# usamec/GAML

Hardware: AMD Instinct MI355X
Metric: reads_per_sec_scored (higher is better)
Workload: dtype f64; 1 GPU; cfg3: 5 Mbp, 50x 2x150 paired, insert 300+-30; 833333 pairs in all, whole true genome as 1-2 walks, 8 rotating path sets, window cache warm; pairs_total=833333, pairs_per_gpu=833333, genome_bp=5000000, parallelism=reads sharded over 1 GPU(s)

## Files before the change

gaml_amd/api.py:

```python
from __future__ import annotations

import ctypes as C
import importlib.util
import os
import sys

import numpy as np

_HERE = os.path.dirname(os.path.abspath(__file__))
FLAVOUR = os.environ.get("GAML_HIP_FLAVOUR", "release")
LIB_PATH = os.environ.get("GAML_HIP_LIB") or os.path.join(_HERE, "libgaml_hip_dev.so" if FLAVOUR == "dev" else "libgaml_hip.so")

OK, EINVAL, ENODEVICE, EHIP, ESTATE = 0, -1, -2, -3, -4

_i32p = np.ctypeslib.ndpointer(np.int32, flags="C_CONTIGUOUS")
_i64p = np.ctypeslib.ndpointer(np.int64, flags="C_CONTIGUOUS")
_f64p = np.ctypeslib.ndpointer(np.float64, flags="C_CONTIGUOUS")
_u8p = np.ctypeslib.ndpointer(np.uint8, flags="C_CONTIGUOUS")

ALIGMENT = np.dtype([("position", np.int32), ("edit_dist", np.int32), ("read_id", np.int32), ("orientation", np.int32)])
PACBIO_ALIGMENT = np.dtype([("position", np.int32), ("position_end", np.int32), ("read_id", np.int32), ("pad_", np.int32),
                            ("logprob", np.float64)])


# ... 88 lines not shown
    L.gaml_hip_add_pacbio_fastq.argtypes = [vp, C.POINTER(SingleCfg), C.c_char_p]
    L.gaml_hip_set_shard.argtypes = [vp, C.c_int32, C.c_int32]
    L.gaml_hip_set_presharded.argtypes = [vp, C.c_int32]
    L.gaml_hip_put_window_records.argtypes = [vp, C.c_int, C.c_int, _i32p, C.c_int32, vp, C.c_int64]
    L.gaml_hip_put_pacbio_records.argtypes = [vp, C.c_int, _i32p, C.c_int32, vp, C.c_int64]
    L.gaml_hip_add_pacbio_reads.argtypes = [vp, C.POINTER(SingleCfg), C.c_int32, _u8p, _i64p, C.c_char_p]
    L.gaml_hip_pacbio_missing.argtypes = [vp, C.c_int, _i32p, C.c_int32, _i32p, C.c_int32]
    L.gaml_hip_pacbio_missing.restype = C.c_int32
    L.gaml_hip_pacbio_ingest_sam.argtypes = [vp, C.c_int, _i32p, C.c_int32, C.c_char_p, C.c_int64, C.POINTER(C.c_int64)]
    L.gaml_hip_pacbio_records.argtypes = [vp, C.c_int, _i32p, C.c_int32, vp, C.c_int64]
    L.gaml_hip_pacbio_records.restype = C.c_int64
    L.gaml_hip_pacbio_dp_stats.argtypes = [vp, C.c_int, _f64p]
    if hasattr(L, "gaml_hip_debug_sam_logprob"):
        L.gaml_hip_debug_sam_logprob.argtypes = [vp, C.c_char_p, C.c_int32, C.c_char_p, C.c_int32, C.c_char_p, C.c_int64, C.c_double, C.POINTER(C.c_double), vp, vp, C.c_int32]
    if hasattr(L, "gaml_hip_debug_sam_shape"):
        L.gaml_hip_debug_sam_shape.argtypes = [C.c_char_p, C.c_int64, C.c_int32, _i32p, C.c_void_p, C.c_int32]
    if hasattr(L, "gaml_hip_debug_sam_band"):
        L.gaml_hip_debug_sam_band.argtypes = [C.c_char_p, C.c_int64, C.c_int32, _i32p, _i32p, _i32p, _i32p, C.c_int32]
        L.gaml_hip_debug_sam_band.restype = C.c_int32
    L.gaml_hip_calc_prob.argtypes = [vp, _i32p, _i64p, C.c_int32, C.POINTER(C.c_double), _i32p, C.POINTER(C.c_int32)]
    L.gaml_hip_calc_prob_batch.argtypes = [vp, C.c_int32, _i32p, _i64p, _i32p, _f64p, vp, vp]
    L.gaml_hip_calc_partials.argtypes = [vp, _i32p, _i64p, C.c_int32, _f64p, C.POINTER(C.c_int32)]
    L.gaml_hip_combine_partials.argtypes = [vp, _f64p, C.c_int32, C.POINTER(C.c_double), _i32p]
    L.gaml_hip_calc_partials_async.argtypes = [vp, _i32p, _i64p, C.c_int32, vp, vp, C.POINTER(C.c_int32)]
    L.gaml_hip_eval_begin.argtypes = [vp, _i32p, _i64p, C.c_int32, C.POINTER(C.c_int64), C.POINTER(C.c_int32)]
    L.gaml_hip_eval_pending_maxpos.argtypes = [vp, vp, C.c_int64]
    L.gaml_hip_eval_pending_maxpos.restype = C.c_int64
    L.gaml_hip_eval_apply_maxpos.argtypes = [vp, _i32p, C.c_int64]
    L.gaml_hip_eval_finish.argtypes = [vp, _f64p]
    L.gaml_hip_eval_finish_async.argtypes = [vp, vp, vp]
    L.gaml_hip_sync.argtypes = [vp]
    L.gaml_hip_compact_tables.argtypes = [vp]
    L.gaml_hip_eval_score_async.argtypes = [vp, vp, vp]
    L.gaml_hip_eval_score_async.restype = C.c_int32
    L.gaml_hip_eval_coverage_export_async.argtypes = [vp, C.c_int32, vp, C.c_int64, C.POINTER(C.c_int64), vp]
    L.gaml_hip_eval_coverage_finish_async.argtypes = [vp, C.c_int32, vp, C.c_int32, C.c_int32, vp]
    L.gaml_hip_eval_pacbio_pending.argtypes = [vp]
    L.gaml_hip_eval_pacbio_pending.restype = C.c_int32
    L.gaml_hip_eval_pacbio_intervals.argtypes = [vp, C.c_int32]
    L.gaml_hip_eval_pacbio_intervals.restype = C.c_int64
    L.gaml_hip_eval_pacbio_export_async.argtypes = [vp, C.c_int32, vp, C.c_int64, vp]
    L.gaml_hip_eval_pacbio_finish_async.argtypes = [vp, C.c_int32, vp, C.c_int64, C.c_int32, vp]
    L.gaml_hip_num_readsets.argtypes = [vp]
    L.gaml_hip_readset_kind.argtypes = [vp, C.c_int]
    L.gaml_hip_readset_reads.argtypes = [vp, C.c_int]
    L.gaml_hip_readset_reads.restype = C.c_int64
    L.gaml_hip_num_nodes.argtypes = [vp]
    L.gaml_hip_node_len.argtypes = [vp, C.c_int32]
    L.gaml_hip_read_probs.argtypes = [vp, C.c_int, _f64p, C.c_int64]
    L.gaml_hip_bad_bases.argtypes = [vp, C.c_int, C.POINTER(C.c_int64)]
    L.gaml_hip_window_count.argtypes = [vp, C.c_int, C.c_int]
    L.gaml_hip_window_count.restype = C.c_int64
    L.gaml_hip_window_records.argtypes = [vp, C.c_int, C.c_int, _i32p, C.c_int32, vp, C.c_int64]
    L.gaml_hip_window_records.restype = C.c_int64
    L.gaml_hip_align_window.argtypes = [vp, C.c_int, C.c_int, _i32p, C.c_int32]
    L.gaml_hip_align_window.restype = C.c_int64
    if hasattr(L, "gaml_hip_debug_prepare"):
        L.gaml_hip_debug_prepare.argtypes = [vp, _i32p, _i64p, C.c_int32]
    if hasattr(L, "gaml_hip_debug_occurrences"):
        L.gaml_hip_debug_occurrences.argtypes = [vp, C.c_int, C.c_int, _i32p, C.c_int64]
    if hasattr(L, "gaml_hip_debug_occurrences"):
        L.gaml_hip_debug_occurrences.restype = C.c_int64
    if hasattr(L, "gaml_hip_debug_table_occurrences"):
        L.gaml_hip_debug_table_occurrences.argtypes = [vp, C.c_int, C.c_int, _i32p, C.c_int64, _i64p]
    if hasattr(L, "gaml_hip_debug_table_occurrences"):
        L.gaml_hip_debug_table_occurrences.restype = C.c_int64
    if hasattr(L, "gaml_hip_debug_window_walk"):
        L.gaml_hip_debug_window_walk.argtypes = [vp, C.c_int, C.c_int, C.c_int32, _i32p, C.c_int32]
    for new, old in (("gaml_hip_pair_classes", "gaml_hip_debug_class_counts"), ("gaml_hip_last_phases", "gaml_hip_debug_profile"),
                     ("gaml_hip_table_stats", "gaml_hip_debug_table_stats")):
        if not hasattr(L, new) and hasattr(L, old):
            setattr(L, new, getattr(L, old))
    L.gaml_hip_pair_classes.argtypes = [vp, C.c_int, _i64p]
    if hasattr(L, "gaml_hip_debug_fold_check"):
        L.gaml_hip_debug_fold_check.argtypes = [vp, C.c_int, _i64p]
    if hasattr(L, "gaml_hip_debug_radix_sort"):
        L.gaml_hip_debug_radix_sort.argtypes = [vp, C.c_void_p, C.c_void_p, C.c_int64, C.c_int, C.c_int, C.c_void_p]
    if hasattr(L, "gaml_hip_debug_tables_check"):
        L.gaml_hip_debug_tables_check.argtypes = [vp, C.c_int, _i64p]
    if hasattr(L, "gaml_hip_debug_static_check"):
        L.gaml_hip_debug_static_check.argtypes = [vp, C.c_int, _i64p]
    if hasattr(L, "gaml_hip_debug_set_knob"):
        L.gaml_hip_debug_set_knob.argtypes = [vp, C.c_int, C.c_int]
    if hasattr(L, "gaml_hip_shm_exchange_open"):
        L.gaml_hip_shm_exchange_open.argtypes = [vp, C.c_char_p, C.c_int32, C.c_int32, C.c_int32]
        L.gaml_hip_shm_allreduce_sum.argtypes = [vp, C.c_void_p, C.c_int32]
        L.gaml_hip_shm_exchange_close.argtypes = [vp, C.c_int32]
    if hasattr(L, "gaml_hip_fetch_async"):
        L.gaml_hip_fetch_async.argtypes = [vp, C.c_void_p, C.c_int32, C.c_void_p]
        L.gaml_hip_fetch_wait.argtypes = [vp, C.c_void_p, C.c_int32]
    if hasattr(L, "gaml_hip_debug_timeline"):
        L.gaml_hip_debug_timeline.argtypes = [vp, C.c_int, C.c_void_p, C.c_int64]
    L.gaml_hip_last_phases.argtypes = [vp, _f64p]
    L.gaml_hip_table_stats.argtypes = [vp, C.c_int, _i64p]
    L.gaml_hip_aligner_stats.argtypes = [vp, C.POINTER(C.c_int64), C.POINTER(C.c_int64), C.POINTER(C.c_double)]
    L.gaml_hip_aligner_stages.argtypes = [vp, _f64p]
    L.gaml_hip_last_timing.argtypes = [vp, _f64p]
    L.gaml_hip_set_event_timing.argtypes = [vp, C.c_int]
    L.gaml_hip_kernel_stats.argtypes = [vp, C.c_int, C.POINTER(C.c_int64), C.POINTER(C.c_double), C.POINTER(C.c_double)]
    return L


_lib = _load()

def lib():
    return _lib


def version() -> str:
    return _lib.gaml_hip_version().decode()


class FlatPaths:

    def __init__(self, paths):
        self.flat, self.offs = _flat(paths)
        self.n = len(paths)
        self.flat_ptr, self.offs_ptr = self.flat.ctypes.data, self.offs.ctypes.data

    def __len__(self):
        return self.n


def _flat(paths):
    if isinstance(paths, FlatPaths):
        return paths.flat, paths.offs
    flat = np.array([x for p in paths for x in p], dtype=np.int32)
    if flat.size == 0:
        flat = np.zeros(1, np.int32)
    offs = np.zeros(len(paths) + 1, dtype=np.int64)
    offs[1:] = np.cumsum([len(p) for p in paths])
    return flat, offs


def comm_unique_id() -> bytes:
    buf = C.create_string_buffer(128)
    rc = _lib.gaml_hip_comm_unique_id(C.cast(buf, C.c_void_p))
    if rc != OK:
        raise GamlHipError(rc, "gaml_hip_comm_unique_id failed (RCCL not loadable?)")
    return buf.raw


class Context:

    def __init__(self, device: int = 0, rank: int = 0, world: int = 1, presharded: int = 1, devices=None):
        self._h = C.c_void_p()
        if devices is not None:
            devs = np.ascontiguousarray(devices, np.int32)
            rc = _lib.gaml_hip_create_multi(C.byref(self._h), devs, len(devs))
            if rc != OK:
                raise GamlHipError(rc, f"gaml_hip_create_multi(devices={list(devs)}) failed")
            device = int(devs[0])
        else:
            rc = _lib.gaml_hip_create(C.byref(self._h), device)
            if rc != OK:
                raise GamlHipError(rc, f"gaml_hip_create(device={device}) failed")
        self.device = device
        if world != 1:
            self._check(_lib.gaml_hip_set_shard(self._h, rank, world))
        elif presharded != 1:
            self._check(_lib.gaml_hip_set_presharded(self._h, presharded))
        self.rank, self.world = rank, world
        self._fast = None
        self._fast_begin = None
        self._fast_combine = None

# ... 326 lines not shown
        _lib.gaml_hip_window_records(self._h, rs, mate, walk, len(walk), out.ctypes.data, n)
        o = out[:n]
        return np.stack([o["position"], o["edit_dist"], o["read_id"], o["orientation"]], axis=1)

    def align_window(self, rs, mate, walk) -> int:
        walk = np.ascontiguousarray(walk, np.int32)
        return _lib.gaml_hip_align_window(self._h, rs, mate, walk, len(walk))

    def debug_prepare(self, paths):
        flat, offs = _flat(paths)
        self._check(_lib.gaml_hip_debug_prepare(self._h, flat, offs, len(paths)))

    def debug_occurrences(self, rs, mate=0) -> np.ndarray:
        n = _lib.gaml_hip_debug_occurrences(self._h, rs, mate, np.zeros(5, np.int32), 0)
        out = np.zeros(5 * max(1, n), np.int32)
        _lib.gaml_hip_debug_occurrences(self._h, rs, mate, out, n)
        return out.reshape(-1, 5)[:n]

    def debug_table_occurrences(self, rs, mate=0):
        info = np.zeros(3, np.int64)
        n = _lib.gaml_hip_debug_table_occurrences(self._h, rs, mate, np.zeros(5, np.int32), 0, info)
        out = np.zeros(5 * max(1, n), np.int32)
        _lib.gaml_hip_debug_table_occurrences(self._h, rs, mate, out, n, info)
        return out.reshape(-1, 5)[:n], {"incremental": bool(info[0]), "incremental_calls": int(info[1]), "full_calls": int(info[2])}

    def debug_window_walk(self, rs, mate, wid) -> list:
        buf = np.zeros(64, np.int32)
        n = _lib.gaml_hip_debug_window_walk(self._h, rs, mate, wid, buf, 64)
        if n > 64:
            buf = np.zeros(n, np.int32)
            _lib.gaml_hip_debug_window_walk(self._h, rs, mate, wid, buf, n)
        return [int(x) for x in buf[:n]]

    def table_stats(self, rs):
        out = np.zeros(10, np.int64)
        self._check(_lib.gaml_hip_table_stats(self._h, rs, out))
        return {"full_rebuilds": int(out[0]), "delta_updates": int(out[1]), "dirty_pairs": int(out[2]), "worker_rebuilds": int(out[3]), "side_stream_rebuilds": int(out[3]),
                "batches_patched": int(out[4]), "batches_full": int(out[5]), "records_left_out": [int(out[6]), int(out[7])], "delta_records_left_out": int(out[8]),
                "static_index_pairs": int(out[9])}

    def aligner_stats(self):
        w, k, us = C.c_int64(), C.c_int64(), C.c_double()
        _lib.gaml_hip_aligner_stats(self._h, C.byref(w), C.byref(k), C.byref(us))
        return {"windows": w.value, "candidates": k.value, "us": us.value}

    def aligner_stages(self):
        out = np.zeros(6, np.float64)
        self._check(_lib.gaml_hip_aligner_stages(self._h, out))
        return {"strings_upload": out[0], "spans_candidates": out[1], "extension": out[2], "hits_d2h": out[3], "sort_file": out[4], "batches": int(out[5])}

    def last_phases(self):
        out = np.zeros(8, np.float64)
        _lib.gaml_hip_last_phases(self._h, out)
        return out

    def debug_timeline(self, rs: int, cap_waves: int = 1 << 16) -> np.ndarray:
        out = np.zeros((cap_waves, 8), np.uint64)
        n = self._check(_lib.gaml_hip_debug_timeline(self._h, rs, out.ctypes.data, cap_waves))
        return out[:n]

    def debug_set_knob(self, knob, value):
        self._check(_lib.gaml_hip_debug_set_knob(self._h, knob, value))

    def debug_fold_check(self, rs):
        out = np.zeros(6, np.int64)
        self._check(_lib.gaml_hip_debug_fold_check(self._h, rs, out))
        return {"records_left_out": [int(out[0]), int(out[1])], "compact_pairs": [int(out[2]), int(out[3])], "records_checked": int(out[4]),
                "violations": int(out[5])}

    def debug_radix_sort(self, keys, vals=None, begin_bit=0, end_bit=64, running_max=False):
        k = np.ascontiguousarray(keys, np.uint64).copy()
        v = None if vals is None else np.ascontiguousarray(vals, np.uint64).copy()
        m = np.zeros(len(k), np.uint64) if running_max else None
        self._check(_lib.gaml_hip_debug_radix_sort(self._h, k.ctypes.data, None if v is None else v.ctypes.data, len(k), begin_bit, end_bit,
                                                   None if m is None else m.ctypes.data))
        return k, v, m

    def debug_static_check(self, rs):
        out = np.zeros(8, np.int64)
        self._check(_lib.gaml_hip_debug_static_check(self._h, rs, out))
        return {"static_pairs": int(out[0]), "other_pairs": int(out[1]), "violations": int(out[2]), "no_record": int(out[3]),
                "different_windows": int(out[4]), "orientation": int(out[5]), "distance": int(out[6]), "edits_or_code": int(out[7])}

    def debug_tables_check(self, rs):
        out = np.zeros(8, np.int64)
        rc = _lib.gaml_hip_debug_tables_check(self._h, rs, out)
        res = {"pairs": int(out[0]), "compact": int(out[1]), "static": int(out[2]), "two": int(out[3]), "four": int(out[4]), "more": int(out[5]),
               "compared": int(out[6]), "mismatches": int(out[7])}
        if rc != 0 and res["compared"] == 0:
            self._check(rc)
        return res

    def debug_block_partials(self, rs, set_index=0):
        sums, zeros, lay = np.zeros(8192, np.float64), np.zeros(8192, np.int32), np.zeros(8, np.int32)
        _lib.gaml_hip_debug_block_partials.argtypes = [C.c_void_p, C.c_int, C.c_int32, _f64p, _i32p, C.c_int32, _i32p]
        n = _lib.gaml_hip_debug_block_partials(self._h, rs, set_index, sums, zeros, 8192, lay)
        return sums[:max(n, 0)].copy(), zeros[:max(n, 0)].copy(), lay.tolist()

    def pair_classes(self, rs):
        out = np.zeros(4, np.int64)
        self._check(_lib.gaml_hip_pair_classes(self._h, rs, out))
        return out

    debug_table_stats, debug_profile, debug_class_counts = table_stats, last_phases, pair_classes

    def last_timing(self):
        out = np.zeros(3, np.float64)
        _lib.gaml_hip_last_timing(self._h, out)
        return {"host_us": out[0], "device_wall_us": out[1], "kernel_us": out[2]}

    def set_event_timing(self, on):
        _lib.gaml_hip_set_event_timing(self._h, int(on))

    def kernel_stats(self, reset=False):
        n, us, b = C.c_int64(), C.c_double(), C.c_double()
        _lib.gaml_hip_kernel_stats(self._h, 1 if reset else 0, C.byref(n), C.byref(us), C.byref(b))
        return {"launches": n.value, "device_us": us.value, "algo_bytes": b.value}


def debug_sam_band(sam_line: str, total_len: int):
    raw = sam_line.encode()
    f = np.zeros(10, np.int32); r0 = np.zeros(1, np.int32)
    n = _lib.gaml_hip_debug_sam_band(raw, len(raw), total_len, f, r0, np.zeros(1, np.int32), np.zeros(1, np.int32), 0)
    if n < 0:
        raise GamlHipError(n, "malformed SAM line")
    lo = np.zeros(n, np.int32); hi = np.zeros(n, np.int32)
    _lib.gaml_hip_debug_sam_band(raw, len(raw), total_len, f, r0, lo, hi, n)
    keys = ["flags", "len", "posstart", "posend", "sstart", "send", "slen", "tstart", "tend", "edit_dist"]
    return dict(zip(keys, (int(x) for x in f))), int(r0[0]), lo, hi


def debug_sam_shape(sam_line: str, total_len: int):
    raw = sam_line.encode()
    f = np.zeros(6, np.int32)
    n = _lib.gaml_hip_debug_sam_shape(raw, len(raw), total_len, f, None, 0)
    if n < 0:
        raise GamlHipError(n, "malformed SAM line")
    ops = np.zeros(max(1, n), np.uint32)
    _lib.gaml_hip_debug_sam_shape(raw, len(raw), total_len, f, ops.ctypes.data, n)
    keys = ["n_ops", "row_f", "col_f", "bl", "el", "max_width"]
    return dict(zip(keys, (int(x) for x in f))), [(int(o) >> 2, "MID"[int(o) & 3]) for o in ops[:n]]
```

gaml_amd/csrc/ctx.hip.h:

```cpp
#pragma once
#include <hip/hip_runtime.h>
#include <hip/hip_ext.h>
#include "radix_sort.hip.h"

#include <algorithm>
#include <atomic>
#include <fcntl.h>
#include <sys/mman.h>
#include <unistd.h>
#include <chrono>
#include <climits>
#include <limits>
#include <cmath>
#include <cstdio>
#include <cstdlib>
#include <cstring>
#include <immintrin.h>
#include <memory>
#include <set>
#include <string>
#include <thread>
#include <vector>

#include "aligner.hip.h"
// ... 162 lines not shown
  DevBuf rec8[2], first[2], extra[2], inl[2], len_code, len12, static_idx, static_val;
  DevBuf slot_of_read, read_of_slot, dirty_of_slot;
  DevBuf cnt;
  bool built = false;
  int64_t class_count[4] = {0, 0, 0, 0}, n0a = 0, extras[2] = {0, 0}, dropped[2] = {0, 0};
  bool keep_dominated = false;
  std::vector<int32_t> read_of_slot_host;
  bool ros_valid = false;
  void release() {
    for (int m = 0; m < 2; m++) { rec8[m].release(); first[m].release(); extra[m].release(); inl[m].release(); }
    len_code.release(); len12.release(); static_idx.release(); static_val.release(); slot_of_read.release(); read_of_slot.release(); dirty_of_slot.release(); cnt.release();
  }
};

struct BuildScratch {
  DevBuf k_in, k_out, k_tmp, v_in, v_tmp, hist, v_sorted[2], rstart[2], rend[2], one[2], cl, sidx, more[2], start[2], tiles, wins[2], peer0;
  PinBuf h_wins[2], h_peer, h_cnt;
  void release() {
    k_in.release(); k_out.release(); k_tmp.release(); v_in.release(); v_tmp.release(); hist.release(); cl.release(); sidx.release(); tiles.release(); peer0.release();
    for (int m = 0; m < 2; m++) { v_sorted[m].release(); rstart[m].release(); rend[m].release(); one[m].release(); more[m].release(); start[m].release(); wins[m].release(); h_wins[m].release(); }
    h_peer.release(); h_cnt.release();
  }
};

struct BuildPlan { int64_t A[2] = {0, 0}; int n_act[2] = {0, 0}; unsigned tiles = 0, none1 = 0, none2 = 0; int ins_n = 0, units = 1; bool empty = true; };

struct TableRebuild {
  bool active = false;
  bool retired = false;
  int next_slice = 0;
  int64_t start_eval = 0;
  TableDev tab;
  hipStream_t stream = nullptr;
  hipEvent_t done = nullptr, mark = nullptr;
  std::vector<std::pair<int32_t, int32_t>> after;
};

struct PairInfo {
  int64_t class_count[4] = {0, 0, 0, 0};
  int64_t n0a = 0;
  std::vector<uint32_t> len_combo;
  int64_t dropped_records[2] = {0, 0};
};

struct PairedSet {
  gaml_paired_cfg cfg;
  ShortMate mate[2];
  PairInfo pt;
  MateDev dev[2];
  TableDev tab;
  TableRebuild rebuild;
  BuildScratch scratch;
  BuildPlan build_plan;
  int64_t async_rebuilds = 0, retired_windows = 0, eval_count = 0;
  DevBuf lcode, len_combo_dev, combo_tabs, memo;
  int memo_codes = 0;
  bool statics_uploaded = false, kernels_warm = false, prereserved = false;
  DevBuf dl_slot, dl_spill, dl_rec[2], sp_rng[2], sp_rec[2], sp_slot, dstate;
  DevBuf dl_bins, dl_bin_count, dl_blk_tot, dl_wlist, dl_stamps;
  PinBuf h_dstate;
  size_t delta_cap = 0, cap_spill = 0, cap_sprec = 0;
  int64_t nd_est = 0, ns_est = 0;
  bool spill_may_grow = false;
  int dl_seq = 0;
  int64_t full_rebuilds = 0, delta_updates = 0;
  int quiet_calls = 0;
  int64_t delta_left_out = 0, delta_left_out_base = 0;
  bool compact_requested = false;
  PinBuf h_timeline; int timeline_waves = 0;
  PinBuf h_part_sum, h_part_zero;
  size_t host_part_stride = 0;
  int last_total_blocks = 0, last_sets = 1;
  int last_blocks[8] = {0, 0, 0, 0, 0, 0, 0, 0};
  bool last_host_partials = false;
  DevBuf probs, tabs, cov_bits, bad;
  Arena arena;
  struct Persist {
    void* dev = nullptr; size_t bytes = 0;
    size_t cap_w[2] = {0, 0}, cap_lo[2] = {0, 0}, cap_m[2] = {0, 0};
    size_t off_tfloor = 0, off_occ[2] = {0, 0}, off_lo[2] = {0, 0}, off_m[2] = {0, 0};
    bool valid = false;
    void release() { if (dev) (void)hipFree(dev); dev = nullptr; bytes = 0; valid = false; }
  } persist;
  int64_t batches_patched = 0, batches_full = 0;
  size_t batch_slack = 0;
  hipEvent_t ev_tables = nullptr, ev_ovf = nullptr;
  PairedPlanner planner;
  OccImage image[2];
  std::vector<Occ> scratch_occ[2];
  Reducer red;
  Staging stage_pool;
  std::vector<double> ins_tab, floor_tab, logfloor_tab, covthr_tab;
  bool floor_positive = true;
  bool tabs_uploaded = false;
  int64_t last_bad_bases = 0;
};

struct SingleSet {
  gaml_single_cfg cfg;
  ShortMate mate;
  ReadMajor rm;
  MateDev dev;
  DevBuf lens, probs, tabs, occ_arena;
  std::vector<Occ> last_occ;
  Reducer red;
  std::vector<double> floor_tab, logfloor_tab;
  bool tabs_uploaded = false;
  Staging stage;
};

struct DpDev {
  DevBuf path, jobs, ops, scratch, out, dbg;
  void release() { path.release(); jobs.release(); ops.release(); scratch.release(); out.release(); dbg.release(); }
};

struct PbSweepDev {
  DevBuf iv_off, iv;
  std::vector<int32_t> iv_off_host;
  uint64_t generation = ~0ull;
  DevBuf in, all;
  DevBuf key_begin, key_end, pos, key_begin_s, key_end_s, pos_s, end_max, tmp, bad;
  Staging stage;
  void release() {
    iv_off.release(); iv.release(); in.release(); all.release(); key_begin.release(); key_end.release(); pos.release();
    key_begin_s.release(); key_end_s.release(); pos_s.release(); end_max.release(); tmp.release(); bad.release();
    for (int k = 0; k < kRing; k++) { stage.host[k].release(); if (stage.done[k]) (void)hipEventDestroy(stage.done[k]); stage.done[k] = nullptr; stage.armed[k] = false; }
  }
};

struct PacbioSet {
  gaml_single_cfg cfg;
  int64_t n_global = 0, lo = 0, hi = 0;
  std::vector<int32_t> lens;
  double log_match = 0, log_mismatch = 0;
  std::unordered_map<Walk, int32_t, WalkHasher> walk_id;
  std::vector<std::vector<gaml_pacbio_aligment>> recs;
  uint64_t generation = 0, uploaded_generation = ~0ull;
  int32_t max_len = 0;
  int64_t misses = 0;
  DevBuf d_lens, rec_off, rec_walk, rec_logp, walk_count, logprobs;
  Reducer red;
  int64_t last_bad_bases = 0;
  Staging stage;
  PbSweepDev sweep;
  bool have_reads = false;
  std::string bases;
  std::vector<int64_t> base_off;
  std::unordered_map<std::string, int32_t> name_id;
  DevBuf d_bases;
  DpDev dp;
  bool bases_uploaded = false;
  double dp_stats[8] = {0, 0, 0, 0, 0, 0, 0, 0};
};

struct PairedPrep {
  int64_t assembled_records = 0;
  std::vector<int32_t> path_base, start_off, starts;
  int32_t total_bits = 0, n_paths = 0;
  bool general = false;
};

struct SetRef { int kind, idx; };

}
}

using namespace gaml;
using namespace gaml::detail;

struct gaml_hip_ctx {
  gaml::MultiState* multi = nullptr;
  gaml::CommState* comm = nullptr;
  int device = -1;
  DevBuf warm_buf; bool general_warm = false;
  AlnJob aln_job[2];
  hipStream_t stream = nullptr;
  hipStream_t aux_stream = nullptr;
  GraphStore g;
  bool have_graph = false;
  std::vector<std::unique_ptr<SingleSet>> singles;
  std::vector<std::unique_ptr<PairedSet>> paireds;
  std::vector<std::unique_ptr<PacbioSet>> pacbios;
  std::vector<SetRef> handles;
  int32_t rank = 0, world = 1;
  AlignScratch aln_scratch;
  AlignSmall aln_small[2];
  int64_t aln_windows = 0, aln_candidates = 0;
  double aln_us = 0;
  double aln_stage_us[5] = {0, 0, 0, 0, 0};
  int64_t aln_batches = 0;
  int knobs[24] = {0};
  bool direct_write = false;
  int32_t peers = 1;
  std::string err;
  bool event_timing = false;
  int event_every = 1;
  int64_t event_tick = 0;
  std::vector<std::pair<hipEvent_t, hipEvent_t>> ev_pool;
  std::vector<uint64_t> ev_call;
  uint64_t eval_serial = 0;
  size_t ev_used = 0;
  double t_host_us = 0, t_dev_wall_us = 0, t_kernel_us = 0;
  int64_t stat_launches = 0;
  double stat_device_us = 0, stat_algo_bytes = 0;
  DevBuf packed;
  PinBuf packed_host;
  char* shm_base = nullptr; size_t shm_bytes = 0; int shm_rank = 0, shm_world = 0, shm_cap = 0; unsigned long long shm_step = 0; std::string shm_name;
  PinBuf fetch_host;
  unsigned long long fetch_seq = 0;
  hipStream_t fetch_stream = nullptr;
  DevBuf batch_dev;
  PinBuf batch_host;
  bool pending_open = false;
  std::vector<Walk> pending_paths;
  bool pending_paths_valid = false;
  int32_t pending_total_len = 0;
  std::vector<std::unique_ptr<PairedPrep>> pending_prep;
  double pending_host_us = 0;
  double prof[8] = {0, 0, 0, 0, 0, 0, 0, 0};
  bool used_default_stream = false;
  double* status_dst = nullptr; double status_a = 0, status_b = 0; bool status_done = false;
  bool host_results = false;
  bool defer_cov = false;
  struct PendingCov { int paired_idx; CovArgs args; double* out4; };
  std::vector<PendingCov> pending_cov;
  struct PendingPacbio {
    int pacbio_idx;
    double* out4;
    int32_t n_paths;
    int64_t n_node, n_own;
  };
  std::vector<PendingPacbio> pending_pb;
};
```

gaml_amd/csrc/debug_api.hip.h:

```cpp
#pragma once

int gaml_hip_debug_prepare(gaml_hip_ctx* c, const int32_t* flat, const int64_t* offs, int32_t n_paths) {
  if (!c || n_paths < 0 || (n_paths > 0 && (!flat || !offs))) return fail(c, GAML_HIP_EINVAL, "bad arguments");
  if (c->multi) {
    for (int k = 0; k < gaml::multi_num_shards(c->multi); k++)
      if (int e = gaml_hip_debug_prepare(gaml::multi_shard(c->multi, k), flat, offs, n_paths)) return fail(c, e, gaml_hip_last_error(gaml::multi_shard(c->multi, k)));
    return GAML_HIP_OK;
  }
  if (!c->have_graph) return fail(c, GAML_HIP_ESTATE, "no graph set");
  std::vector<Walk> paths = unflatten(flat, offs, n_paths);
  for (auto& h : scoring_order(c)) {
    if (h.kind == 0) { std::vector<Occ> occs; prepare_single_host(c, *c->singles[h.idx], paths, occs); }
    else if (h.kind == 1) {
      PairedPrep p;
      PairedSet& ps = *c->paireds[h.idx];
      if (int e = prepare_paired_structure(c, ps, flat, offs, n_paths)) return e;
      if (int e = align_pending_pair(c, ps)) return e;
      prepare_paired_tables_host(c, ps, p);
    }
  }
  if (c->peers == 1) {
    for (ShortMate* m : filter_mates(c)) m->unsynced.clear();
  }
  return GAML_HIP_OK;
}

int64_t gaml_hip_debug_occurrences(gaml_hip_ctx* c, int rs, int mate, int32_t* out5, int64_t cap) {
  MULTI_SHARD0(c);
  if (!c || rs < 0 || rs >= (int)c->handles.size()) return -1;
  SetRef h = c->handles[rs];
  const std::vector<Occ>* v = nullptr;
  if (h.kind == 0) v = &c->singles[h.idx]->last_occ;
  else if (h.kind == 1 && (mate == 0 || mate == 1)) { PairedSet& ps = *c->paireds[h.idx]; ps.planner.flat_occurrences(mate, ps.scratch_occ[mate]); v = &ps.scratch_occ[mate]; }
  if (!v) return -1;
  for (int64_t i = 0; i < (int64_t)v->size() && i < cap; i++) {
    const Occ& o = (*v)[i];
    out5[5 * i] = o.wid; out5[5 * i + 1] = o.shift; out5[5 * i + 2] = o.min_pos; out5[5 * i + 3] = o.path; out5[5 * i + 4] = o.rank;
  }
  return (int64_t)v->size();
}

int64_t gaml_hip_debug_table_occurrences(gaml_hip_ctx* c, int rs, int mate, int32_t* out5, int64_t cap, int64_t* info3) {
  MULTI_SHARD0(c);
  if (!c || rs < 0 || rs >= (int)c->handles.size() || c->handles[rs].kind != 1 || (mate != 0 && mate != 1)) return -1;
  PairedSet& ps = *c->paireds[c->handles[rs].idx];
  if (info3) { info3[0] = ps.planner.last_was_incremental(); info3[1] = (int64_t)ps.planner.incremental_calls; info3[2] = (int64_t)ps.planner.full_calls; }
  std::vector<Occ> v;
  ps.image[mate].dump(v);
  const std::vector<int32_t>& slots = ps.planner.slots();
  std::unordered_map<int32_t, int32_t> pos;
  for (size_t k = 0; k < slots.size(); k++) pos[slots[k]] = (int32_t)k;
  for (Occ& o : v) { auto it = pos.find(o.path); o.path = it == pos.end() ? -1 : it->second; }
  std::sort(v.begin(), v.end(), [](const Occ& a, const Occ& b) { return a.path != b.path ? a.path < b.path : (a.rank != b.rank ? a.rank < b.rank : a.wid < b.wid); });
  for (int64_t i = 0; i < (int64_t)v.size() && i < cap; i++) {
    const Occ& o = v[(size_t)i];
    out5[5 * i] = o.wid; out5[5 * i + 1] = o.shift; out5[5 * i + 2] = o.min_pos; out5[5 * i + 3] = o.path; out5[5 * i + 4] = o.rank;
  }
  return (int64_t)v.size();
}

int32_t gaml_hip_debug_window_walk(gaml_hip_ctx* c, int rs, int mate, int32_t wid, int32_t* out, int32_t cap) {
  MULTI_SHARD0(c);
  ShortMate* m = mate_of(c, rs, mate);
  if (!m || wid < 0 || wid >= (int32_t)m->win_walk.size()) return -1;
  const Walk& w = *m->win_walk[wid];
  for (int32_t i = 0; i < (int32_t)w.size() && i < cap; i++) out[i] = w[i];
  return (int32_t)w.size();
}



int gaml_hip_debug_timeline(gaml_hip_ctx* c, int rs, unsigned long long* out, int64_t cap_waves) {
  MULTI_SHARD0(c);
  if (!c || rs < 0 || rs >= (int)c->handles.size() || c->handles[rs].kind != 1 || !out) return fail(c, GAML_HIP_EINVAL, "bad arguments");
  PairedSet& s = *c->paireds[c->handles[rs].idx];
  if (!s.h_timeline.p) return 0;
  const int64_t n = std::min<int64_t>(cap_waves, s.timeline_waves);
  memcpy(out, s.h_timeline.p, (size_t)n * 8 * sizeof(unsigned long long));
  return (int)n;
}

int gaml_hip_debug_set_knob(gaml_hip_ctx* c, int knob, int value) {
  if (!c || knob < 0 || knob >= 24) return GAML_HIP_EINVAL;
  if (c->multi) { for (int k = 0; k < gaml::multi_num_shards(c->multi); k++) gaml::multi_shard(c->multi, k)->knobs[knob] = value; return GAML_HIP_OK; }
  c->knobs[knob] = value;
  return GAML_HIP_OK;
}


static void paired_base_records(const PairTables& pt, int32_t slot, int mt, std::vector<RecQuad>& out) {
  const int64_t n0s = pt.class_count[0];
  if (slot < n0s) {
    const uint64_t r = pt.rec8[mt][slot];
    if (r != kNoRec8) out.push_back(RecQuad{(int32_t)(r & 0xffffff), (int32_t)((r >> 24) & 0xfffffff), (int32_t)((r >> 52) & 63) | ((int32_t)((r >> 58) & 1) << 8), 0});
  } else {
    const RecQuad& f = pt.rm[mt].first[slot - n0s];
    if (f.wid >= 0) {
      const int cnt1 = 1 + (int)((uint32_t)f.flags >> 9);
      for (int q = 0; q < cnt1; q++) { RecQuad r = q == 0 ? f : pt.rm[mt].extra[f.link + q - 1]; r.flags &= 0x1ff; r.link = 0; out.push_back(r); }
    }
  }
}

int gaml_hip_debug_fold_check(gaml_hip_ctx* c, int rs, int64_t* out6) {
  MULTI_SHARD0(c);
  if (!c || rs < 0 || rs >= (int)c->handles.size() || c->handles[rs].kind != 1 || !out6) return fail(c, GAML_HIP_EINVAL, "bad arguments");
  PairedSet& s = *c->paireds[c->handles[rs].idx];
  for (int mt = 0; mt < 2; mt++) for (const Window& w : s.mate[mt].wins) if (w.first < 0 && w.count > 0) return fail(c, GAML_HIP_ESTATE, "host-only check: some windows' records exist in the device pool only (use gaml_hip_debug_tables_check)");
  PairTables with, without;
  build_pair_tables(s.mate[0], s.mate[1], with, true);
  build_pair_tables(s.mate[0], s.mate[1], without, false);
  int64_t checked = 0, bad = 0;
  const int64_t n = s.mate[0].n_local();
  std::vector<RecQuad> a, b;
  for (int mt = 0; mt < 2; mt++) {
    const ShortMate& m = s.mate[mt];
    for (int64_t read = 0; read < n; read++) {
      a.clear(); b.clear();
      paired_base_records(with, with.slot_of_read[read], mt, a);
      paired_base_records(without, without.slot_of_read[read], mt, b);
      size_t ia = 0;
      for (size_t ib = 0; ib < b.size(); ib++) {
        checked++;
        const RecQuad& r = b[ib];
        if (ia < a.size() && a[ia].wid == r.wid && a[ia].pos == r.pos && a[ia].flags == r.flags) { ia++; continue; }
        const Window& j = m.wins[r.wid];
        bool ok = false;
        if (j.head >= 0) {
          auto it = m.solo_of_node.find(j.head);
          if (it != m.solo_of_node.end() && m.wins[it->second].active)
// ... 88 lines not shown
  if (!s.last_host_partials || set < 0 || set >= kMaxSets) return 0;
  const int n = s.last_blocks[set];
  const double* hs = (const double*)s.h_part_sum.p + (size_t)set * s.host_part_stride;
  const int* hz = (const int*)s.h_part_zero.p + (size_t)set * s.host_part_stride;
  for (int b = 0; b < n && b < cap; b++) { if (sums) sums[b] = hs[b]; if (zeros) zeros[b] = hz[b]; }
  if (layout8) {
    PairedArgs a; GridPlan gp;
    paired_base_args(c, s, a, gp);
    layout8[0] = gp.blocks0a; layout8[1] = gp.blocks0; layout8[2] = a.blocks01; layout8[3] = a.blocks012; layout8[4] = a.main_blocks; layout8[5] = a.total_blocks;
    layout8[6] = 0; layout8[7] = n;
  }
  return n;
}



int gaml_hip_debug_tables_check(gaml_hip_ctx* c, int rs, int64_t* out8) {
  MULTI_SHARD0(c);
  if (!c || rs < 0 || rs >= (int)c->handles.size() || c->handles[rs].kind != 1 || !out8) return fail(c, GAML_HIP_EINVAL, "bad arguments");
  if (c->device < 0) return fail(c, GAML_HIP_ENODEVICE, "host-only context");
  PairedSet& s = *c->paireds[c->handles[rs].idx];
  HIP_TRY(c, hipSetDevice(c->device));
  if (s.rebuild.active) { if (int e = paired_build_continue(c, s, true)) return e; HIP_TRY(c, hipEventSynchronize(s.rebuild.done)); s.rebuild.active = false; s.rebuild.after.clear(); }
  if (int e = prepare_paired_tables(c, s)) return e;
  if (int e = pool_mirror(c, s, c->stream)) return e;
  if (int e = paired_upload_statics(c, s, c->stream)) return e;
  TableDev T;
  if (int e = paired_build_enqueue(c, s, T, c->stream)) return e;
  HIP_TRY(c, hipStreamSynchronize(c->stream));
  if (int e = paired_build_collect(c, s, T)) { T.release(); return e; }
  ShortMate hm[2];
  for (int mt = 0; mt < 2; mt++) {
    const ShortMate& m = s.mate[mt];
    hm[mt].n_global = m.n_global; hm[mt].lo = m.lo; hm[mt].hi = m.hi; hm[mt].lens = m.lens;
    hm[mt].wins = m.wins;
    std::vector<int4> dp((size_t)s.dev[mt].pool_n);
    if (!dp.empty()) HIP_TRY(c, hipMemcpy(dp.data(), s.dev[mt].pool.p, dp.size() * sizeof(int4), hipMemcpyDeviceToHost));
    hm[mt].pool.resize(dp.size());
    for (size_t k = 0; k < dp.size(); k++) hm[mt].pool[k] = gaml_aligment{dp[k].y, dp[k].z & 0xff, dp[k].w, (dp[k].z >> 8) & 1};
    for (Window& w : hm[mt].wins) w.first = w.dfirst < 0 ? 0 : w.dfirst;
    for (Window& w : hm[mt].wins) if (w.dfirst < 0) { w.count = 0; }
  }
  PairTables pt;
  build_pair_tables(hm[0], hm[1], pt, KNOB(c, 16) != 1, paired_static_ins_n(c, s));
  const int64_t n = s.mate[0].n_local();
  int64_t compared = 0, bad = 0;
  auto fetch = [&](const DevBuf& d, size_t bytes, std::vector<char>& out) -> int {
    out.resize(bytes);
    if (bytes) HIP_TRY(c, hipMemcpy(out.data(), d.p, bytes, hipMemcpyDeviceToHost));
    return 0;
  };
  auto cmp = [&](const DevBuf& d, const void* host, size_t bytes, size_t elem, const char* what) -> int {
    std::vector<char> v;
    if (int e = fetch(d, bytes, v)) return e;
    int64_t b0 = bad;
    for (size_t k = 0; k < bytes / elem; k++) { compared++; if (memcmp(v.data() + k * elem, (const char*)host + k * elem, elem) != 0) bad++; }
    if (bad != b0 && getenv("GAML_HIP_TRACE_HOST")) fprintf(stderr, "tables_check: %s differs in %lld of %zu entries\n", what, (long long)(bad - b0), bytes / elem);
    return 0;
  };
  for (int k = 0; k < 4; k++) { compared++; bad += T.class_count[k] != pt.class_count[k]; }
  compared++; bad += T.n0a != pt.n0a;
  if (bad == 0) {
    const int64_t n0 = pt.class_count[0], n16 = n - n0;
    if (int e = cmp(T.slot_of_read, pt.slot_of_read.data(), (size_t)n * 4, 4, "slot_of_read")) return e;
    if (int e = cmp(T.read_of_slot, pt.read_of_slot.data(), (size_t)n * 4, 4, "read_of_slot")) return e;
    for (int mt = 0; mt < 2; mt++) {
      if (int e = cmp(T.rec8[mt], pt.rec8[mt].data(), (size_t)n0 * 8, 8, "rec8")) return e;
      if (int e = cmp(T.first[mt], pt.rm[mt].first.data(), (size_t)n16 * 16, 16, "first")) return e;
      if (int e = cmp(T.extra[mt], pt.rm[mt].extra.data(), pt.rm[mt].extra.size() * 16, 16, "extra")) return e;
      if (int e = cmp(T.inl[mt], pt.inl[mt].data(), pt.inl[mt].size() * 16, 16, "inl")) return e;
      compared++; bad += T.extras[mt] != (int64_t)pt.rm[mt].extra.size();
      compared++; bad += T.dropped[mt] != pt.dropped_records[mt];
    }
    if (int e = cmp(T.len_code, pt.len_code.data(), (size_t)n0, 1, "len_code")) return e;
    if (int e = cmp(T.static_idx, pt.static_idx.data(), (size_t)pt.n0a * 4, 4, "static_idx")) return e;
    if (int e = cmp(T.len12, pt.len12.data(), (size_t)n16 * 4, 4, "len12")) return e;
    compared++; bad += pt.len_combo != s.pt.len_combo;
  }
  out8[0] = n; out8[1] = T.class_count[0]; out8[2] = T.n0a; out8[3] = T.class_count[1]; out8[4] = T.class_count[2]; out8[5] = T.class_count[3];
  out8[6] = compared; out8[7] = bad;
  T.release();
  return bad ? fail(c, GAML_HIP_ESTATE, "record tables: the device build differs from the host restatement") : GAML_HIP_OK;
}
```

gaml_amd/csrc/gaml_hip.hip:

```cpp
#include "ctx.hip.h"

using namespace gaml;
using namespace gaml::detail;

namespace {

namespace {
struct KernargEnv {
  bool was_set;
  KernargEnv() { was_set = getenv("HIP_FORCE_DEV_KERNARG") != nullptr; setenv("HIP_FORCE_DEV_KERNARG", "1", 0); }
} kernarg_env;
}

int fail(gaml_hip_ctx* c, int code, const std::string& msg) {
  if (c) c->err = msg;
  return code;
}
#define HIP_TRY(c, expr)                                                                      \
  do {                                                                                        \
    hipError_t e__ = (expr);                                                                  \
    if (e__ != hipSuccess)                                                                    \
      return fail(c, GAML_HIP_EHIP, std::string(#expr) + ": " + hipGetErrorString(e__));      \
  } while (0)

// ... 98 lines not shown
  if (c->ev_used == c->ev_pool.size() && c->ev_pool.size() >= 2048) { if (int e = collect_events(c)) return e; }
  if (c->ev_used == c->ev_pool.size()) {
    hipEvent_t a, b;
    HIP_TRY(c, hipEventCreate(&a));
    HIP_TRY(c, hipEventCreate(&b));
    c->ev_pool.emplace_back(a, b);
  }
  if (c->ev_call.size() < c->ev_pool.size()) c->ev_call.resize(c->ev_pool.size(), 0);
  c->ev_call[c->ev_used] = c->eval_serial;
  *out = &c->ev_pool[c->ev_used++];
  return 0;
}

struct OccLayout { size_t direct, multi_off, multi, end; };
OccLayout layout_image(const OccImage& t, size_t at, size_t n_entries = 0) {
  OccLayout l;
  l.direct = at;
  l.multi_off = (l.direct + std::max<size_t>(1, std::max(n_entries, t.occ12.size())) * sizeof(Occ12) + 15) & ~(size_t)15;
  l.multi = (l.multi_off + t.multi_off.size() * sizeof(int32_t) + 15) & ~(size_t)15;
  l.end = (l.multi + std::max<size_t>(1, t.multi.size()) * sizeof(OccQuad) + 15) & ~(size_t)15;
  return l;
}
void pack_image(const OccImage& t, const OccLayout& l, char* base) {
  if (!t.occ12.empty()) memcpy(base + l.direct, t.occ12.data(), t.occ12.size() * sizeof(Occ12));
  const size_t used = l.direct + t.occ12.size() * sizeof(Occ12);
  if (l.multi_off > used) memset(base + used, 0xff, l.multi_off - used);
  memcpy(base + l.multi_off, t.multi_off.data(), t.multi_off.size() * sizeof(int32_t));
  if (!t.multi.empty()) memcpy(base + l.multi, t.multi.data(), t.multi.size() * sizeof(OccQuad));
}
OccLayout layout_occ(const OccTable& t, size_t at) {
  OccLayout l;
  l.direct = at;
  l.multi_off = align16(l.direct + std::max<size_t>(1, t.direct.size()) * sizeof(OccQuad));
  l.multi = align16(l.multi_off + t.multi_off.size() * sizeof(int32_t));
  l.end = align16(l.multi + std::max<size_t>(1, t.multi.size()) * sizeof(OccQuad));
  return l;
}
void pack_occ(const OccTable& t, const OccLayout& l, char* base) {
  if (!t.direct.empty()) memcpy(base + l.direct, t.direct.data(), t.direct.size() * sizeof(OccQuad));
  memcpy(base + l.multi_off, t.multi_off.data(), t.multi_off.size() * sizeof(int32_t));
  if (!t.multi.empty()) memcpy(base + l.multi, t.multi.data(), t.multi.size() * sizeof(OccQuad));
}

int upload_mate(gaml_hip_ctx* c, const ShortMate& m, ReadMajor& rm, MateDev& d, hipStream_t st,
                const std::vector<int32_t>* slot_of_read = nullptr, bool force = false) {
  if (d.pow_n == 0) {
    d.pow_n = m.match_pow.size();
    HIP_TRY(c, d.pows.reserve(2 * d.pow_n * sizeof(double)));
    HIP_TRY(c, hipMemcpy(d.pows.p, m.mismatch_pow.data(), d.pow_n * sizeof(double), hipMemcpyHostToDevice));
    HIP_TRY(c, hipMemcpy(d.pows.as<double>() + d.pow_n, m.match_pow.data(), d.pow_n * sizeof(double), hipMemcpyHostToDevice));
  }
  if (d.uploaded_generation == m.active_generation && !force) return 0;
  build_read_major(m, slot_of_read, rm);
  HIP_TRY(c, hipStreamSynchronize(st));
  HIP_TRY(c, d.first.reserve(std::max<size_t>(1, rm.first.size()) * sizeof(RecQuad)));
  HIP_TRY(c, d.extra.reserve(std::max<size_t>(1, rm.extra.size()) * sizeof(RecQuad)));
  if (!rm.first.empty()) HIP_TRY(c, hipMemcpy(d.first.p, rm.first.data(), rm.first.size() * sizeof(RecQuad), hipMemcpyHostToDevice));
  if (!rm.extra.empty()) HIP_TRY(c, hipMemcpy(d.extra.p, rm.extra.data(), rm.extra.size() * sizeof(RecQuad), hipMemcpyHostToDevice));
  d.uploaded_generation = m.active_generation;
  return 0;
}

MateView view_of(const MateDev& d, const char* arena, const OccLayout& l) {
  MateView v;
  v.first = d.first.as<int4>();
  v.extra = d.extra.as<int4>();
  v.occ = (const int4*)(arena + l.direct);
  v.occ12 = nullptr;
  v.multi_off = (const int*)(arena + l.multi_off);
  v.multi = (const int4*)(arena + l.multi);
  v.mism_pow = d.pows.as<double>();
  v.match_pow = d.pows.as<double>() + d.pow_n;
  return v;
}

std::vector<Walk> unflatten(const int32_t* flat, const int64_t* offs, int32_t n) {
  std::vector<Walk> r(n);
  for (int32_t i = 0; i < n; i++) r[i].assign(flat + offs[i], flat + offs[i + 1]);
  return r;
}

}

#include "paired_launch.hip.h"

namespace {

#include "single_launch.hip.h"
#include "pacbio_launch.hip.h"
#include "aligner_launch.hip.h"
std::vector<ShortMate*> filter_mates(gaml_hip_ctx* c) {
  std::vector<ShortMate*> v;
  for (auto& h : c->handles)
    if (h.kind == 1) { v.push_back(&c->paireds[h.idx]->mate[0]); v.push_back(&c->paireds[h.idx]->mate[1]); }
  return v;
}

int eval_begin(gaml_hip_ctx* c, const int32_t* flat, const int64_t* offs, int32_t n_paths, int64_t* pending) {
  if (!c->have_graph) return fail(c, GAML_HIP_ESTATE, "no graph set");
  if (n_paths < 0 || (n_paths > 0 && (!flat || !offs))) return fail(c, GAML_HIP_EINVAL, "bad path arguments");
  const double t0 = now_us();
  c->eval_serial++;
  for (int32_t i = 0; i < n_paths; i++) if (offs[i + 1] < offs[i]) return fail(c, GAML_HIP_EINVAL, "path offsets must not decrease");
  const bool want_vectors = c->paireds.empty() || !c->singles.empty() || !c->pacbios.empty();
  c->pending_paths_valid = want_vectors;
  if (want_vectors) {
    c->pending_paths.resize((size_t)n_paths);
    for (int32_t i = 0; i < n_paths; i++) c->pending_paths[i].assign(flat + offs[i], flat + offs[i + 1]);
    for (auto& p : c->pending_paths)
      for (int32_t x : p)
        if (x >= c->g.n()) return fail(c, GAML_HIP_EINVAL, "path refers to a node outside the graph");
    c->pending_total_len = 0;
    for (auto& p : c->pending_paths) c->pending_total_len += walk_length(c->g, p);
  }
  if (c->pending_prep.size() != c->paireds.size()) { c->pending_prep.clear(); c->pending_prep.resize(c->paireds.size()); }
  for (size_t i = 0; i < c->paireds.size(); i++) {
    if (!c->pending_prep[i]) c->pending_prep[i].reset(new PairedPrep());
    if (int e = prepare_paired_structure(c, *c->paireds[i], flat, offs, n_paths)) return e;
    if (!want_vectors) c->pending_total_len = c->paireds[i]->planner.total_len();
    const double ta = now_us();
    gpu_probe(c->stream, c->warm_buf.p, "before alignment");
    if (int e = align_pending_pair(c, *c->paireds[i])) return e;
    gpu_probe(c->stream, c->warm_buf.p, "after alignment");
    c->prof[2] = (i ? c->prof[2] : 0.0) + now_us() - ta;
  }
  int64_t n = 0;
  for (ShortMate* m : filter_mates(c)) {
    if (c->peers == 1) m->unsynced.clear();
    n += (int64_t)m->unsynced.size();
  }
  for (auto& s : c->singles) s->mate.unsynced.clear();
  if (pending) *pending = n;
  gpu_probe(c->stream, c->warm_buf.p, "end of eval_begin");
  c->pending_open = true;
  c->pending_host_us = now_us() - t0;
  c->prof[0] = c->pending_host_us;
  return 0;
}

int eval_finish(gaml_hip_ctx* c, void* d_partials, hipStream_t st) {
  if (c->device < 0) return fail(c, GAML_HIP_ENODEVICE, "scoring needs a HIP device: this context is host-only");
  if (!c->pending_open) return fail(c, GAML_HIP_ESTATE, "no evaluation in progress");
  for (ShortMate* m : filter_mates(c))
    if (!m->unsynced.empty())
      return fail(c, GAML_HIP_ESTATE, "sharded context: new windows were aligned; exchange their largest positions "
                                      "(gaml_hip_eval_pending_maxpos -> all-reduce(max) -> gaml_hip_eval_apply_maxpos) before finishing");
  if (c->peers > 1) {
    for (auto& ps : c->paireds)
      if (ps->cfg.penalty_constant > 0 && !c->defer_cov)
        return fail(c, GAML_HIP_ESTATE, "penalty_constant > 0 on a sharded context: the coverage maps of all ranks must be merged "
                                        "(gaml_hip_eval_score_async -> gaml_hip_eval_coverage_export_async -> all-gather -> "
                                        "gaml_hip_eval_coverage_finish_async)");
    for (auto& ps : c->pacbios)
      if (ps->cfg.penalty_constant > 0 && !c->defer_cov)
        return fail(c, GAML_HIP_ESTATE, "penalty_constant > 0 on a sharded PacBio set: the alignment intervals of all ranks must be merged "
                                        "(gaml_hip_eval_score_async -> gaml_hip_eval_pacbio_export_async -> all-gather -> gaml_hip_eval_pacbio_finish_async)");
  }
  const std::vector<Walk>& paths = c->pending_paths;
  const int32_t total_len = c->pending_total_len;
  auto order = scoring_order(c);
  const double t0 = now_us();
  c->t_host_us = 0;
  int k = 0;
  for (auto& h : order) {
    const double tk = now_us();
    double* out4 = (double*)d_partials + 4 * k;
// ... 95 lines not shown
void ctx_eval_abandon(gaml_hip_ctx* c) { if (c) { c->pending_open = false; c->pending_cov.clear(); c->pending_pb.clear(); } }
bool ctx_has_penalty(const gaml_hip_ctx* c) {
  for (auto& ps : c->paireds) if (ps->cfg.penalty_constant > 0) return true;
  for (auto& ps : c->pacbios) if (ps->cfg.penalty_constant > 0) return true;
  return false;
}
}

#define MULTI_FWD(c, call) do { if ((c) && (c)->multi) return gaml::call; } while (0)
#define MULTI_SHARD0(c) do { if ((c) && (c)->multi) (c) = gaml::multi_shard((c)->multi, 0); } while (0)
#define MULTI_REFUSE(c, what) do { if ((c) && (c)->multi) return fail(c, GAML_HIP_ESTATE, "multi-device context: " what); } while (0)

extern "C" {


int gaml_hip_create(gaml_hip_ctx** out, int device) {
  if (!out) return GAML_HIP_EINVAL;
  *out = nullptr;
  std::unique_ptr<gaml_hip_ctx> c(new gaml_hip_ctx());
  c->device = device;
  if (device >= 0) {
    int count = 0;
    hipError_t e = hipGetDeviceCount(&count);
    if (e != hipSuccess || device >= count) {
      fprintf(stderr, "gaml_hip_create: HIP device %d not available (%s)\n", device, e == hipSuccess ? "ordinal out of range" : hipGetErrorString(e));
      return GAML_HIP_ENODEVICE;
    }
    if (hipSetDevice(device) != hipSuccess) return GAML_HIP_EHIP;
    {
      const char* ka = getenv("HIP_FORCE_DEV_KERNARG");
      static bool warned = false;
      if ((!ka || strcmp(ka, "1") != 0) && !warned) {
        warned = true;
        c->err = "HIP_FORCE_DEV_KERNARG is not 1: kernel arguments live in host memory, every scoring launch pays ~4 us for it";
        fprintf(stderr, "libgaml_hip: warning: %s\n", c->err.c_str());
      }
    }
    {
      int lo = 0, hi = 0;
      if (hipDeviceGetStreamPriorityRange(&lo, &hi) != hipSuccess || hipStreamCreateWithPriority(&c->stream, hipStreamNonBlocking, hi) != hipSuccess) return GAML_HIP_EHIP;
    }
    if (hipStreamCreateWithFlags(&c->aux_stream, hipStreamNonBlocking) != hipSuccess) return GAML_HIP_EHIP;
    int large_bar = 0;
    if (hipDeviceGetAttribute(&large_bar, hipDeviceAttributeIsLargeBar, device) != hipSuccess) large_bar = 0;
    const char* dw = getenv("GAML_HIP_DIRECT_WRITE");
    c->direct_write = large_bar != 0 && !(dw && dw[0] == '0');
  }
  *out = c.release();
  return GAML_HIP_OK;
}

void gaml_hip_destroy(gaml_hip_ctx* c) {
#ifdef GAML_GEN_STAMPS
  if (c && c->device >= 0) {
    unsigned long long z[32];
    if (hipMemcpyFromSymbol(z, HIP_SYMBOL(gaml::g_gen_stamp), sizeof(z)) == hipSuccess && z[15]) {
      fprintf(stderr, "general_pair_staged: longest stage us: entries %.1f, bounds %.1f, lists %.1f, liveness %.1f, terms %.1f; waves above 10 us in a stage: %llu %llu %llu %llu %llu\n",
              z[16] * 0.01, z[17] * 0.01, z[18] * 0.01, z[19] * 0.01, z[20] * 0.01, z[24], z[25], z[26], z[27], z[28]);
    }
    if (z[6]) fprintf(stderr, "general_pair_call as the caller sees it: %llu calls, mean %.2f us; from the class body's entry to the call %.2f us\n", z[6], z[5] * 0.01 / z[6], z[21] * 0.01 / z[6]);
    if (z[15])
      fprintf(stderr, "general_pair_staged: %llu waves; mean us per wave: entries %.2f, bounds %.2f, lists %.2f, liveness %.2f, terms %.2f; candidates per lane-0 pair %.1f / %.1f, live %.1f, lanes %.1f; pairs that did not fit %llu; longest %.2f us, most candidates %llu / %llu, most live %llu / %llu\n",
              z[15], z[0] * 0.01 / z[15], z[1] * 0.01 / z[15], z[2] * 0.01 / z[15], z[3] * 0.01 / z[15], z[4] * 0.01 / z[15], (double)z[8] / z[15], (double)z[9] / z[15], (double)z[10] / z[15], (double)z[11] / z[15], z[12], z[13] * 0.01, z[14] / 1000, z[14] % 1000, z[7] / 1000, z[7] % 1000);
  }
#endif
  if (c && c->shm_base) { munmap(c->shm_base, c->shm_bytes); c->shm_base = nullptr; }
  if (!c) return;
  if (c->multi) { gaml::multi_destroy(c->multi); c->multi = nullptr; }
  if (c->device >= 0) {
    (void)hipSetDevice(c->device);
    (void)hipDeviceSynchronize();
    if (c->comm) { gaml::comm_destroy(c->comm); c->comm = nullptr; }
    auto drop_stage = [](Staging& s) { for (int k = 0; k < kRing; k++) { s.host[k].release(); if (s.done[k]) (void)hipEventDestroy(s.done[k]); } };
    for (auto& s : c->singles) { s->dev.first.release(); s->dev.extra.release(); s->dev.pows.release(); s->lens.release(); s->probs.release(); s->tabs.release(); s->occ_arena.release(); s->red.release(); drop_stage(s->stage); }
    for (auto& s : c->paireds) {
      if (s->rebuild.stream) (void)hipStreamDestroy(s->rebuild.stream);
      if (s->rebuild.done) (void)hipEventDestroy(s->rebuild.done);
      if (s->rebuild.mark) (void)hipEventDestroy(s->rebuild.mark);
      s->tab.release(); s->rebuild.tab.release(); s->scratch.release();
      for (int m = 0; m < 2; m++) { s->dev[m].first.release(); s->dev[m].extra.release(); s->dev[m].pows.release(); s->dev[m].aln.release(); s->dev[m].pool.release(); s->dev[m].lens.release();
                                    s->dl_rec[m].release(); s->sp_rng[m].release(); s->sp_rec[m].release(); }
      s->dl_slot.release(); s->dl_spill.release(); s->sp_slot.release(); s->dstate.release(); s->dl_bins.release(); s->dl_bin_count.release(); s->dl_blk_tot.release(); s->dl_wlist.release(); s->h_dstate.release(); s->lcode.release(); s->len_combo_dev.release(); s->combo_tabs.release(); s->memo.release();
      drop_stage(s->stage_pool); s->h_part_sum.release(); s->h_part_zero.release(); s->h_timeline.release();
      s->probs.release(); s->tabs.release(); s->arena.release(); s->persist.release(); s->cov_bits.release(); s->bad.release(); if (s->ev_tables) (void)hipEventDestroy(s->ev_tables); if (s->ev_ovf) (void)hipEventDestroy(s->ev_ovf);
      s->red.release();
    }
    for (auto& s : c->pacbios) { s->d_lens.release(); s->rec_off.release(); s->rec_walk.release(); s->rec_logp.release(); s->walk_count.release(); s->logprobs.release(); s->red.release(); drop_stage(s->stage);
      s->d_bases.release(); s->dp.release(); s->sweep.release(); }
    c->packed.release(); c->packed_host.release(); c->batch_dev.release(); c->batch_host.release(); c->aln_scratch.release();
    c->aln_small[0].release(); c->aln_small[1].release(); c->fetch_host.release(); c->warm_buf.release();
    for (auto& e : c->ev_pool) { (void)hipEventDestroy(e.first); (void)hipEventDestroy(e.second); }
    if (c->stream) (void)hipStreamDestroy(c->stream);
    if (c->aux_stream) (void)hipStreamDestroy(c->aux_stream);
  }
  delete c;
}

const char* gaml_hip_last_error(const gaml_hip_ctx* c) {
  if (!c) return "null context";
  if (c->multi && c->err.empty()) return gaml::multi_last_error(c->multi);
  return c->err.c_str();
}

int gaml_hip_set_graph(gaml_hip_ctx* c, int32_t n_nodes, const char* bases, const int64_t* offs) {
  if (!c || n_nodes < 0 || !offs || (n_nodes > 0 && !bases)) return fail(c, GAML_HIP_EINVAL, "bad graph arguments");
  if (n_nodes & 1) return fail(c, GAML_HIP_EINVAL, "node count must be even (twin of i is i^1)");
  MULTI_FWD(c, multi_set_graph(c->multi, n_nodes, bases, offs));
  c->g.bases.assign(bases + offs[0], bases + offs[n_nodes]);
  c->g.off.resize(n_nodes + 1);
  for (int32_t i = 0; i <= n_nodes; i++) c->g.off[i] = offs[i] - offs[0];
  c->g.finish();
  c->have_graph = true;
  return GAML_HIP_OK;
}

int gaml_hip_load_graph(gaml_hip_ctx* c, const char* file) {
  if (!c || !file) return fail(c, GAML_HIP_EINVAL, "bad arguments");
  MULTI_FWD(c, multi_load_graph(c->multi, file));
  std::string err;
  if (!c->g.load_lastgraph(file, &err)) return fail(c, GAML_HIP_EINVAL, err);
  c->have_graph = true;
  return GAML_HIP_OK;
}

int gaml_hip_set_shard(gaml_hip_ctx* c, int32_t rank, int32_t world) {
  if (!c || world < 1 || rank < 0 || rank >= world) return fail(c, GAML_HIP_EINVAL, "bad shard");
  MULTI_REFUSE(c, "its shards are the devices given to gaml_hip_create_multi");
  if (!c->handles.empty()) return fail(c, GAML_HIP_ESTATE, "set the shard before adding read sets");
  c->rank = rank; c->world = world; c->peers = world;
  return GAML_HIP_OK;
}

int gaml_hip_set_presharded(gaml_hip_ctx* c, int32_t world) {
  if (!c || world < 1) return fail(c, GAML_HIP_EINVAL, "bad arguments");
  MULTI_REFUSE(c, "its shards are the devices given to gaml_hip_create_multi");
  if (c->world != 1) return fail(c, GAML_HIP_ESTATE, "gaml_hip_set_shard already partitions this context's reads");
  c->peers = world;
  return GAML_HIP_OK;
}

static void init_mate(gaml_hip_ctx* c, ShortMate& m, double mismatch, int64_t n, const char* b, const int64_t* offs) {
  m.mismatch = mismatch;
  m.match = 1.0 - 4 * mismatch;
  int64_t lo, hi;
  shard_range(c, n, &lo, &hi);
  m.set_reads(n, lo, hi, b, offs);
}

int gaml_hip_add_single(gaml_hip_ctx* c, const gaml_single_cfg* cfg, int32_t n, const char* bases, const int64_t* offs) {
  if (!c || !cfg || n < 0 || !offs) return fail(c, GAML_HIP_EINVAL, "bad arguments");
  MULTI_FWD(c, multi_add_single(c->multi, cfg, n, bases, offs));
  std::unique_ptr<SingleSet> s(new SingleSet());
  s->cfg = *cfg;
  init_mate(c, s->mate, cfg->mismatch_prob, n, bases, offs);
  c->singles.push_back(std::move(s));
  c->handles.push_back(SetRef{0, (int)c->singles.size() - 1});
  return (int)c->handles.size() - 1;
}

static int warm_general_kernels(gaml_hip_ctx* c) {
  if (c->general_warm || c->device < 0) return 0;
  HIP_TRY(c, hipSetDevice(c->device));
  HIP_TRY(c, c->warm_buf.reserve(256));
  HIP_TRY(c, hipMemsetAsync(c->warm_buf.p, 0, 256, c->stream));
  PairedArgs a;
  memset((void*)&a, 0, sizeof(a));
  a.total_blocks = 1;
// ... 370 lines not shown
  MULTI_REFUSE(c, "no single device to fetch from");
  if (c->device < 0) return fail(c, GAML_HIP_ENODEVICE, "no device");
  HIP_TRY(c, hipSetDevice(c->device));
  const size_t bytes = 512 + (size_t)n_doubles * sizeof(double);
  if (bytes > c->fetch_host.cap) {
    HIP_TRY(c, c->fetch_host.reserve(bytes));
    memset(c->fetch_host.p, 0, c->fetch_host.cap);
  }
  c->fetch_stream = caller_stream(c, stream);
  c->fetch_seq++;
  char* dev = (char*)c->fetch_host.dev;
  hipLaunchKernelGGL(fetch_kernel, dim3(1), dim3(64), 0, c->fetch_stream, (const double*)d_src, (int)n_doubles, (double*)(dev + 512),
                     (unsigned long long*)dev, c->fetch_seq);
  HIP_TRY(c, hipGetLastError());
  return GAML_HIP_OK;
}

int gaml_hip_fetch_wait(gaml_hip_ctx* c, double* out, int32_t n_doubles) {
  if (!c || !out || n_doubles <= 0 || !c->fetch_host.p) return fail(c, GAML_HIP_EINVAL, "bad arguments / no fetch in flight");
  volatile unsigned long long* word = (volatile unsigned long long*)c->fetch_host.p;
  const double t0 = now_us();
  bool seen = false;
  while (now_us() - t0 < 2000.0) {
    for (int k = 0; k < 64 && !seen; k++) seen = *word == c->fetch_seq;
    if (seen) break;
  }
  if (!seen) {
    HIP_TRY(c, hipSetDevice(c->device));
    HIP_TRY(c, hipStreamSynchronize(c->fetch_stream));
    if (*word != c->fetch_seq) return fail(c, GAML_HIP_ESTATE, "fetch kernel finished without publishing its sequence word");
  }
  std::atomic_thread_fence(std::memory_order_acquire);
  memcpy(out, (const char*)c->fetch_host.p + 512, (size_t)n_doubles * sizeof(double));
  return GAML_HIP_OK;
}

int gaml_hip_sync(gaml_hip_ctx* c) {
  MULTI_FWD(c, multi_sync(c->multi));
  if (!c || c->device < 0) return fail(c, GAML_HIP_ENODEVICE, "no device");
  HIP_TRY(c, hipSetDevice(c->device));
  HIP_TRY(c, hipStreamSynchronize(c->stream));
  if (c->used_default_stream) { HIP_TRY(c, hipStreamSynchronize(nullptr)); c->used_default_stream = false; }
  for (auto& ps : c->paireds) paired_refresh_counts(*ps);
  return GAML_HIP_OK;
}

static int fetch_partials(gaml_hip_ctx* c, double* partials_out);

int gaml_hip_eval_finish(gaml_hip_ctx* c, double* partials_out) {
  if (!c || !partials_out) return fail(c, GAML_HIP_EINVAL, "bad arguments");
  MULTI_REFUSE(c, "the gaml_hip_eval_* protocol is for one shard per process");
  if (c->device < 0) return fail(c, GAML_HIP_ENODEVICE, "scoring needs a HIP device: this context is host-only");
  HIP_TRY(c, hipSetDevice(c->device));
  const size_t bytes = std::max<size_t>(1, c->handles.size()) * 4 * sizeof(double);
  HIP_TRY(c, c->packed_host.reserve(bytes));
  void* dres = nullptr;
  HIP_TRY(c, hipHostGetDevicePointer(&dres, c->packed_host.p, 0));
  c->host_results = true;
  int e = eval_finish(c, dres, c->stream);
  c->host_results = false;
  if (e) return e;
  return fetch_partials(c, partials_out);
}

int gaml_hip_calc_partials_async(gaml_hip_ctx* c, const int32_t* paths, const int64_t* offs, int32_t n_paths,
                                 void* d_partials, void* stream, int32_t* total_len_out) {
  if (!c || !d_partials) return fail(c, GAML_HIP_EINVAL, "bad arguments");
  MULTI_REFUSE(c, "partials of several devices have no single device address; use gaml_hip_calc_partials");
  if (c->device >= 0) HIP_TRY(c, hipSetDevice(c->device));
  return evaluate(c, paths, offs, n_paths, d_partials, caller_stream(c, stream), total_len_out);
}

int gaml_hip_calc_partials(gaml_hip_ctx* c, const int32_t* paths, const int64_t* offs, int32_t n_paths,
                           double* partials_out, int32_t* total_len_out) {
  if (!c || !partials_out) return fail(c, GAML_HIP_EINVAL, "bad arguments");
  MULTI_FWD(c, multi_calc_partials(c->multi, paths, offs, n_paths, partials_out, total_len_out));
  if (c->device < 0) return fail(c, GAML_HIP_ENODEVICE, "scoring needs a HIP device: this context is host-only");
  HIP_TRY(c, hipSetDevice(c->device));
  const size_t bytes = std::max<size_t>(1, c->handles.size()) * 4 * sizeof(double);
  HIP_TRY(c, c->packed_host.reserve(bytes));
  void* dres = nullptr;
  HIP_TRY(c, hipHostGetDevicePointer(&dres, c->packed_host.p, 0));
  c->host_results = true;
  int e = evaluate(c, paths, offs, n_paths, dres, c->stream, total_len_out);
  c->host_results = false;
  if (e) return e;
  return fetch_partials(c, partials_out);
}

static void finisher_order_sum(const double* ps, const int* pz, int n, double* sum_out, double* zeros_out) {
  double v[kBlock];
  long long z = 0;
  for (int t = 0; t < kBlock; t++) { double a = 0; for (int b = t; b < n; b += kBlock) a += ps[b]; v[t] = a; }
  for (int b = 0; b < n; b++) z += pz[b];
  double total = 0;
  for (int w = 0; w < kBlock / 64; w++) {
    double* l = v + 64 * w;
    for (int off = 32; off > 0; off >>= 1) for (int i = 0; i < off; i++) l[i] += l[i + off];
    total += l[0];
  }
  *sum_out = total;
  *zeros_out = (double)z;
}

static int wait_host_partials(gaml_hip_ctx* c, bool* spun) {
  const double t0 = now_us();
  bool spin = KNOB(c, 7) == 0 && !c->handles.empty();
  for (auto& h : c->handles) if (h.kind != 1) spin = false;
  for (auto& ps : c->paireds) if (ps->cfg.penalty_constant > 0 || !ps->last_host_partials || ps->last_total_blocks == 0) spin = false;
  if (spin) {
    const double deadline = t0 + 2e6;
    for (auto& ps : c->paireds) {
      for (int k = 0; k < ps->last_sets && spin; k++) {
        const volatile double* hs = (const volatile double*)ps->h_part_sum.p + (size_t)k * ps->host_part_stride;
        const volatile int* hz = (const volatile int*)ps->h_part_zero.p + (size_t)k * ps->host_part_stride;
        int done = 0;
        while (done < ps->last_blocks[k]) {
          if (hs[done] == hs[done] && hz[done] != INT_MIN) { done++; continue; }
          __builtin_ia32_pause();
          if ((done & 63) == 0 && now_us() > deadline) { spin = false; break; }
        }
      }
      if (!spin) break;
    }
    std::atomic_thread_fence(std::memory_order_acquire);
  }
  if (!spin) HIP_TRY(c, hipStreamSynchronize(c->stream));
  c->t_dev_wall_us += now_us() - t0;
  c->prof[7] = now_us() - t0;
  *spun = spin;
  return 0;
}

static int fetch_partials(gaml_hip_ctx* c, double* partials_out) {
  bool spun = false;
  if (int e = wait_host_partials(c, &spun)) return e;
  {
    double* res = (double*)c->packed_host.p;
    auto ord = scoring_order(c);
    for (size_t k = 0; k < ord.size(); k++) {
      if (ord[k].kind != 1) continue;
      PairedSet& s = *c->paireds[ord[k].idx];
      if (!s.last_host_partials) continue;
      if (s.last_blocks[0] > 0)
        finisher_order_sum((const double*)s.h_part_sum.p, (const int*)s.h_part_zero.p, s.last_blocks[0], &res[4 * k], &res[4 * k + 1]);
      else res[4 * k] = res[4 * k + 1] = 0;
      if (!(s.cfg.penalty_constant > 0) || s.last_total_blocks == 0) res[4 * k + 2] = 0;
      res[4 * k + 3] = (double)s.mate[0].n_local();
    }
  }
  memcpy(partials_out, c->packed_host.p, c->handles.size() * 4 * sizeof(double));
  for (auto& ps : c->paireds) {
    paired_refresh_counts(*ps);
    if (paired_delta_overflowed(*ps)) return fail(c, GAML_HIP_ESTATE, "delta store overflow (spill area); call gaml_hip_compact_tables and evaluate again");
  }
  c->t_kernel_us = 0;
  if (!spun) { if (int e2 = collect_events(c)) return e2; }
  auto order = scoring_order(c);
  for (size_t k = 0; k < order.size(); k++) {
    if (order[k].kind == 1) c->paireds[order[k].idx]->last_bad_bases = (int64_t)partials_out[4 * k + 2];
    else if (order[k].kind == 2) c->pacbios[order[k].idx]->last_bad_bases = (int64_t)partials_out[4 * k + 2];
  }
  return GAML_HIP_OK;
}

#include "paired_batch.hip.h"
int gaml_hip_combine_partials(gaml_hip_ctx* c, const double* partials, int32_t total_len, double* prob_out, int32_t* zeros_out) {
  if (!c || !partials || !prob_out) return fail(c, GAML_HIP_EINVAL, "bad arguments");
  MULTI_FWD(c, multi_combine(c->multi, partials, total_len, prob_out, zeros_out));
  return combine(c, partials, prob_out, zeros_out, total_len);
}

int gaml_hip_calc_prob(gaml_hip_ctx* c, const int32_t* paths, const int64_t* offs, int32_t n_paths,
                       double* prob_out, int32_t* zeros_out, int32_t* total_len_out) {
  if (!c || !prob_out) return fail(c, GAML_HIP_EINVAL, "bad arguments");
  const size_t ns = c->multi ? (size_t)gaml::multi_num_readsets(c->multi) : c->handles.size();
  std::vector<double> partials(std::max<size_t>(1, ns) * 4);
  int32_t tl = 0;
  int e;
  if (!c->multi && c->comm) {
    e = gaml::comm_eval_reduced(c, paths, offs, n_paths, partials.data(), &tl);
  } else {
    if (c->peers != 1)
      return fail(c, GAML_HIP_ESTATE, "sharded context without a communicator: gaml_hip_comm_init_rank first, or use gaml_hip_calc_partials + "
                                      "your own all-reduce + gaml_hip_combine_partials");
    e = gaml_hip_calc_partials(c, paths, offs, n_paths, partials.data(), &tl);
  }
  if (e) return e;
  if (total_len_out) *total_len_out = tl;
  return gaml_hip_combine_partials(c, partials.data(), tl, prob_out, zeros_out);
}

int gaml_hip_calc_prob_batch(gaml_hip_ctx* c, int32_t n_sets, const int32_t* paths, const int64_t* offs, const int32_t* set_offs,
                             double* probs_out, int32_t* zeros_out, int32_t* total_lens_out) {
  if (!c || n_sets < 0 || !set_offs || !probs_out || (n_sets > 0 && !offs)) return fail(c, GAML_HIP_EINVAL, "bad arguments");
  MULTI_FWD(c, multi_calc_prob_batch(c->multi, n_sets, paths, offs, set_offs, probs_out, zeros_out, total_lens_out));
  if (c->comm && n_sets > 0) {
    const size_t nsr = std::max<size_t>(1, c->handles.size());
    std::vector<double> part((size_t)n_sets * 4 * nsr);
    std::vector<int32_t> tls((size_t)n_sets, 0);
    if (int e = gaml::comm_eval_reduced_batch(c, n_sets, paths, offs, set_offs, part.data(), tls.data())) return e;
    for (int32_t i = 0; i < n_sets; i++) {
      if (int e = combine(c, part.data() + (size_t)i * 4 * nsr, &probs_out[i], zeros_out ? zeros_out + (size_t)i * 2 * nsr : nullptr, tls[i])) return e;
      if (total_lens_out) total_lens_out[i] = tls[i];
    }
    return GAML_HIP_OK;
  }
  if (c->world != 1 || c->peers != 1)
    return fail(c, GAML_HIP_ESTATE, "sharded context without a communicator: gaml_hip_comm_init_rank first, or run the gaml_hip_eval_* protocol per path "
                                    "set and all-reduce the partials of the batch at once");
  if (c->device < 0) return fail(c, GAML_HIP_ENODEVICE, "scoring needs a HIP device: this context is host-only");
  if (n_sets == 0) return GAML_HIP_OK;
  HIP_TRY(c, hipSetDevice(c->device));
  const size_t ns = std::max<size_t>(1, c->handles.size());
  for (int32_t i = 0; i < n_sets; i++) if (set_offs[i + 1] < set_offs[i]) return fail(c, GAML_HIP_EINVAL, "set offsets must not decrease");
  int32_t done_sets = 0;
  if (batch_fast_capable(c)) {
    std::vector<double> part((size_t)kMaxSets * 4 * ns);
    int32_t tls[kMaxSets];
    while (done_sets < n_sets) {
      const int n = std::min<int32_t>(kMaxSets, n_sets - done_sets);
      int rc = n > 1 ? batch_chunk_patched(c, n, paths, offs, set_offs + done_sets, part.data(), tls) : 1;
      if (rc > 0 && n > 1) rc = batch_chunk_fast(c, n, paths, offs, set_offs + done_sets, part.data(), tls);
      if (rc < 0) return rc;
      if (rc > 0) break;
      for (int k = 0; k < n; k++) {
        const int32_t i = done_sets + k;
        if (int e = combine(c, part.data() + (size_t)k * 4 * ns, &probs_out[i], zeros_out ? zeros_out + (size_t)i * 2 * ns : nullptr, tls[k])) return e;
        if (total_lens_out) total_lens_out[i] = tls[k];
      }
      done_sets += n;
    }
    if (done_sets == n_sets) return GAML_HIP_OK;
    set_offs += done_sets; probs_out += done_sets;
    if (zeros_out) zeros_out += (size_t)done_sets * 2 * ns;
    if (total_lens_out) total_lens_out += done_sets;
    n_sets -= done_sets;
  }
  const size_t doubles = (size_t)n_sets * 4 * ns;
  if (doubles * sizeof(double) > c->batch_dev.cap) { HIP_TRY(c, hipStreamSynchronize(c->stream)); HIP_TRY(c, c->batch_dev.reserve(doubles * sizeof(double))); }
  HIP_TRY(c, c->batch_host.reserve(doubles * sizeof(double)));
  std::vector<int32_t> tls(n_sets, 0);
  for (int32_t i = 0; i < n_sets; i++) {
    const int32_t p0 = set_offs[i], p1 = set_offs[i + 1];
    if (p1 < p0) return fail(c, GAML_HIP_EINVAL, "set offsets must not decrease");
    if (int e = evaluate(c, paths, offs + p0, p1 - p0, c->batch_dev.as<double>() + (size_t)i * 4 * ns, c->stream, &tls[i])) {
      (void)hipStreamSynchronize(c->stream);
      return e;
    }
  }
  HIP_TRY(c, hipMemcpyAsync(c->batch_host.p, c->batch_dev.p, doubles * sizeof(double), hipMemcpyDeviceToHost, c->stream));
  HIP_TRY(c, hipStreamSynchronize(c->stream));
  const double* res = (const double*)c->batch_host.p;
  for (int32_t i = 0; i < n_sets; i++) {
    if (int e = combine(c, res + (size_t)i * 4 * ns, &probs_out[i], zeros_out ? zeros_out + (size_t)i * 2 * ns : nullptr, tls[i])) return e;
    if (total_lens_out) total_lens_out[i] = tls[i];
  }
  return GAML_HIP_OK;
}

int gaml_hip_num_readsets(const gaml_hip_ctx* c) { MULTI_FWD(c, multi_num_readsets(c->multi)); return c ? (int)c->handles.size() : 0; }
int gaml_hip_readset_kind(const gaml_hip_ctx* c, int rs) {
  MULTI_FWD(c, multi_readset_kind(c->multi, rs));
  return (c && rs >= 0 && rs < (int)c->handles.size()) ? c->handles[rs].kind : -1;
}
int64_t gaml_hip_readset_reads(const gaml_hip_ctx* c, int rs) {
  MULTI_FWD(c, multi_readset_reads(c->multi, rs));
  if (!c || rs < 0 || rs >= (int)c->handles.size()) return -1;
  SetRef h = c->handles[rs];
  if (h.kind == 0) return c->singles[h.idx]->mate.n_global;
  if (h.kind == 1) return c->paireds[h.idx]->mate[0].n_global;
  return c->pacbios[h.idx]->n_global;
}
int32_t gaml_hip_num_nodes(const gaml_hip_ctx* c) { MULTI_FWD(c, multi_num_nodes(c->multi)); return c && c->have_graph ? c->g.n() : 0; }
int32_t gaml_hip_node_len(const gaml_hip_ctx* c, int32_t node) { MULTI_FWD(c, multi_node_len(c->multi, node)); return (c && c->have_graph && node >= 0 && node < c->g.n()) ? c->g.len(node) : -1; }

int gaml_hip_read_probs(gaml_hip_ctx* c, int rs, double* out, int64_t n) {
  MULTI_FWD(c, multi_read_probs(c->multi, rs, out, n));
  if (!c || rs < 0 || rs >= (int)c->handles.size() || !out) return fail(c, GAML_HIP_EINVAL, "bad arguments");
  if (c->device < 0) return fail(c, GAML_HIP_ENODEVICE, "host-only context");
  SetRef h = c->handles[rs];
  const void* src; int64_t have;
  if (h.kind == 0) { src = c->singles[h.idx]->probs.p; have = c->singles[h.idx]->mate.n_local(); }
  else if (h.kind == 1) { src = c->paireds[h.idx]->probs.p; have = c->paireds[h.idx]->mate[0].n_local(); }
  else { src = c->pacbios[h.idx]->logprobs.p; have = c->pacbios[h.idx]->hi - c->pacbios[h.idx]->lo; }
  if (!src) return fail(c, GAML_HIP_ESTATE, "read set not scored yet");
  if (n < have) return fail(c, GAML_HIP_EINVAL, "output too small");
  HIP_TRY(c, hipSetDevice(c->device));
  HIP_TRY(c, hipDeviceSynchronize());
  if (have) HIP_TRY(c, hipMemcpy(out, src, have * sizeof(double), hipMemcpyDeviceToHost));
  if (h.kind == 1 && have) {
    TableDev& T = c->paireds[h.idx]->tab;
    if (!T.ros_valid) {
      T.read_of_slot_host.resize((size_t)have);
      HIP_TRY(c, hipMemcpy(T.read_of_slot_host.data(), T.read_of_slot.p, (size_t)have * sizeof(int32_t), hipMemcpyDeviceToHost));
      T.ros_valid = true;
// ... 157 lines not shown
```

gaml_amd/csrc/host_model.cc:

```cpp
#include "host_model.h"

#include <algorithm>
#include <chrono>
#include <cmath>
#include <cstdlib>
#include <cstring>
#include <fstream>
#include <thread>

namespace gaml {

void GraphStore::finish() {
  norm.resize(n());
  std::unordered_map<std::string, int32_t> tiny;
  for (int32_t i = 0; i < n(); i++) {
    norm[i] = i;
    if (len(i) > 3) continue;
    std::string s(seq(i), len(i));
    auto it = tiny.find(s);
    if (it == tiny.end()) tiny.emplace(s, i);
    else norm[i] = it->second;
  }
}

// ... 753 lines not shown
          return false;
        }
        memos_[id]->last_used = clock_;
        memos_[id]->use_count++;
        total_len_ += memos_[id]->length;
        in_ids.push_back(id);
        int32_t slot;
        if (!free_slots_.empty()) { slot = free_slots_.back(); free_slots_.pop_back(); }
        else slot = next_slot_++;
        in_slots.push_back(slot);
      }
    free_slots_.insert(free_slots_.end(), freed_now.begin(), freed_now.end());
    {
      size_t taken = in_ids.size();
      for (size_t q = edits_.size(); q-- > 0;) {
        const Edit& e = edits_[q];
        const size_t cnt = (size_t)(e.c1 - e.c0);
        taken -= cnt;
        cur_ids_.erase(cur_ids_.begin() + e.p0, cur_ids_.begin() + e.p1);
        cur_ids_.insert(cur_ids_.begin() + e.p0, in_ids.begin() + taken, in_ids.begin() + taken + cnt);
        cur_slots_.erase(cur_slots_.begin() + e.p0, cur_slots_.begin() + e.p1);
        cur_slots_.insert(cur_slots_.begin() + e.p0, in_slots.begin() + taken, in_slots.begin() + taken + cnt);
      }
    }
    is_new_.assign((size_t)n_paths, 0);
    for (const Edit& e : edits_) for (int32_t k = e.c0; k < e.c1; k++) is_new_[k] = 1;
    for (const Edit& e : edits_) {
      int32_t chain_end = e.c1;
      while (chain_end < n_paths) { const bool has_node = memos_[cur_ids_[chain_end]]->final_last_end != -2; chain_end++; if (has_node) break; }
      registration_chain(g, mate, e.c0, chain_end);
    }
    std::vector<char>& redo = redo_;
    redo.assign(memos_.size(), 0);
    for (int32_t id : in_ids) redo[id] = 1;
    for (int32_t id : stale_) if (id < (int32_t)memos_.size() && memos_[id]->use_count > 0 && (!memos_[id]->valid[0] || !memos_[id]->valid[1] || !memos_[id]->occ_valid[0] || !memos_[id]->occ_valid[1])) redo[id] = 2;
    stale_.clear();
    drain(mate);
    size_t seen = stale_.size();
    for (int32_t k = 0; k < n_paths; k++) {
      const int32_t id = cur_ids_[k];
      if (!redo[id]) continue;
      PathMemo& pm = *memos_[id];
      bool built = false;
      for (int mt = 0; mt < 2; mt++)
        if (!pm.valid[mt]) { build_placements(g, mate[mt], mt, pm, id); built = true; }
      if (!built) continue;
      drain(mate);
      for (; seen < stale_.size(); seen++) {
        const int32_t sid = stale_[seen];
        if (sid >= (int32_t)redo.size() || redo[sid]) continue;
        for (int32_t q = k + 1; q < n_paths; q++) if (cur_ids_[q] == sid) { redo[sid] = 2; break; }
      }
    }
    for (int32_t k = 0; k < n_paths; k++) {
      const int32_t id = cur_ids_[k];
      if (!redo[id]) continue;
      if (!is_new_[k]) {
        const PathMemo& pm = *memos_[id];
        removed_.push_back(Removed{cur_slots_[k], {pm.assembled[0], pm.assembled[1]}, {pm.occ[0], pm.occ[1]}});
      }
      work_.push_back(k);
    }
    std::vector<int32_t> keep;
    for (int32_t sid : stale_) if (sid < (int32_t)memos_.size() && memos_[sid]->use_count > 0 && (!memos_[sid]->valid[0] || !memos_[sid]->valid[1])) keep.push_back(sid);
    stale_.swap(keep);
  }
  const int64_t total = n_paths > 0 ? offs[n_paths] - base : 0;
  prev_flat_.assign(flat + base, flat + base + total);
  prev_offs_.resize((size_t)n_paths + 1);
  for (int32_t k = 0; k <= n_paths; k++) prev_offs_[k] = (n_paths > 0 ? offs[k] : 0) - base;
  have_prev_ = true;
  return true;
}

static void occ_prepack(const std::vector<Occ>& occ, std::vector<OccPre>& pre) {
  pre.resize(occ.size());
  for (size_t k = 0; k < occ.size(); k++) {
    const Occ& o = occ[k];
    const int32_t mp = o.min_pos < -32768 ? -32768 : o.min_pos;
    pre[k] = OccPre{o.min_pos <= 32767 ? o.wid : ~o.wid, (uint32_t)o.shift, (uint32_t)(uint16_t)(int16_t)mp, o.rank};
  }
}

void PairedPlanner::invalidate_thresholds() {
  for (auto& pm : memos_) pm->occ_valid[0] = pm->occ_valid[1] = false;
  have_prev_ = false;
}

void PairedPlanner::finish(ShortMate mate[2]) {
  auto redo_occ = [&](PathMemo& pm) {
    for (int mt = 0; mt < 2; mt++) {
      if (pm.occ_valid[mt]) continue;
      pm.occ[mt].clear();
      occurrences_from_placements(mate[mt], pm.pl[mt], pm.occ[mt]);
      pm.assembled[mt] = 0;
      for (const Occ& o : pm.occ[mt]) pm.assembled[mt] += mate[mt].wins[o.wid].count;
      occ_prepack(pm.occ[mt], pm.pre[mt]);
      pm.occ_valid[mt] = true;
    }
  };
  if (!incremental_) {
    for (int32_t id : cur_ids_) redo_occ(*memos_[id]);
    assembled_[0] = assembled_[1] = 0;
    for (int32_t id : cur_ids_) { assembled_[0] += memos_[id]->assembled[0]; assembled_[1] += memos_[id]->assembled[1]; }
  } else {
    for (int32_t k : work_) redo_occ(*memos_[cur_ids_[k]]);
  }
}

const PlanView& PairedPlanner::view() {
  if (!view_valid_) {
    view_.paths.clear();
    for (int32_t id : cur_ids_) view_.paths.push_back(memos_[id].get());
    view_valid_ = true;
  }
  return view_;
}

void PairedPlanner::apply(ShortMate mate[2], OccImage image[2]) {
  if (!incremental_) {
    const PlanView& v = view();
    for (int32_t id : cur_ids_) {
      PathMemo& pm = *memos_[id];
      if (pm.touched_serial == retire_serial_) continue;
      for (int mt = 0; mt < 2; mt++) for (const Occ& o : pm.occ[mt]) mate[mt].touch(o.wid);
      pm.touched_serial = retire_serial_;
    }
    for (int mt = 0; mt < 2; mt++) image[mt].build(mate[mt].wins.size(), v, mt);
    return;
  }
  for (int32_t k : work_) {
    PathMemo& pm = *memos_[cur_ids_[k]];
    if (pm.touched_serial == retire_serial_) continue;
    for (int mt = 0; mt < 2; mt++) for (const Occ& o : pm.occ[mt]) mate[mt].touch(o.wid);
    pm.touched_serial = retire_serial_;
  }
  if ((int32_t)pos_of_slot_.size() < next_slot_) pos_of_slot_.resize((size_t)next_slot_ + 64, 0);
  for (int32_t k = 0; k < (int32_t)cur_slots_.size(); k++) pos_of_slot_[cur_slots_[k]] = k;
  for (int mt = 0; mt < 2; mt++) {
    OccImage& im = image[mt];
    for (const Removed& r : removed_) { im.remove_path(r.occ[mt], r.slot); assembled_[mt] -= r.assembled[mt]; }
    for (int32_t k : work_) {
      const PathMemo& pm = *memos_[cur_ids_[k]];
      im.add_path(mate[mt].wins.size(), pm.occ[mt], cur_slots_[k]);
      assembled_[mt] += pm.assembled[mt];
    }
    im.finalize(pos_of_slot_);
  }
}

void PairedPlanner::mark_used(ShortMate mate[2], const OccImage image[2]) {
  for (int mt = 0; mt < 2; mt++) image[mt].for_each_present([&](int32_t w) { mate[mt].touch(w); });
  for (auto& pm : memos_)
    if (pm->last_used > rebuild_clock_ || pm->use_count > 0)
      for (int mt = 0; mt < 2; mt++) for (const Occ& o : pm->occ[mt]) if (o.wid < (int32_t)mate[mt].wins.size()) mate[mt].touch(o.wid);
}

void PairedPlanner::flat_occurrences(int mate, std::vector<Occ>& out) {
  out.clear();
  int32_t rank0 = 0;
  const PlanView& v = view();
  for (size_t slot = 0; slot < v.paths.size(); slot++) {
    const PathMemo& pm = *v.paths[slot];
    for (const Occ& o : pm.occ[mate]) out.push_back(Occ{o.wid, o.shift, o.min_pos, (int32_t)slot, rank0 + o.rank});
    rank0 += (int32_t)pm.occ[mate].size();
  }
}

void build_read_major(const ShortMate& m, const std::vector<int32_t>* slot_of_read, ReadMajor& out) {
  const int64_t n = m.n_local();
  auto slot = [&](int32_t read) { return slot_of_read ? (*slot_of_read)[read] : read; };
  std::vector<int32_t> cnt(n + 1, 0);
  for (const Window& w : m.wins) if (w.active) for (int64_t k = w.first; k < w.first + w.count; k++) cnt[slot(m.pool[k].read_id) + 1]++;
  std::vector<int64_t> start(n + 1, 0);
  int64_t extras = 0;
  for (int64_t i = 0; i < n; i++) { start[i] = extras; extras += cnt[i + 1] > 1 ? cnt[i + 1] - 1 : 0; }
  out.first.assign(n, RecQuad{-1, 0, 0, 0});
  out.extra.assign(extras, RecQuad{-1, 0, 0, 0});
  std::vector<int32_t> seen(n, 0);
  for (size_t wid = 0; wid < m.wins.size(); wid++) {
    const Window& win = m.wins[wid];
    if (!win.active) continue;
    for (int64_t k = win.first; k < win.first + win.count; k++) {
      const gaml_aligment& r = m.pool[k];
      const int32_t at = slot(r.read_id);
      RecQuad q{(int32_t)wid, r.position, (r.edit_dist & 0xff) | ((r.orientation & 1) << 8), 0};
      int32_t s = seen[at]++;
      if (s == 0) {
        int32_t more = cnt[at + 1] - 1;
        q.flags |= more << 9;
        q.link = (int32_t)start[at];
        out.first[at] = q;
      } else {
        out.extra[start[at] + s - 1] = q;
      }
    }
  }
  out.total_records = m.active_records;
  out.built_generation = m.active_generation;
}

#ifdef GAML_HIP_DEV
static void dominated_records(const ShortMate& m, std::vector<uint8_t>& drop) {
  drop.assign(m.pool.size(), 0);
  std::unordered_map<int32_t, int32_t> solo;
  bool any_head = false;
  for (size_t wid = 0; wid < m.wins.size(); wid++) {
    const Window& w = m.wins[wid];
    if (!w.active || w.count == 0) continue;
    if (w.solo >= 0) solo.emplace(w.solo, (int32_t)wid);
    any_head |= w.head >= 0;
  }
  if (!any_head || solo.empty()) return;
  auto before = [](const gaml_aligment& x, const gaml_aligment& y) { return x.position != y.position ? x.position < y.position : x.read_id < y.read_id; };
  for (const Window& j : m.wins) {
    if (!j.active || j.count == 0 || j.head < 0) continue;
    auto it = solo.find(j.head);
    if (it == solo.end()) continue;
    const Window& sw = m.wins[it->second];
    const gaml_aligment* a = m.pool.data() + j.first, * const ae = a + j.count;
    const gaml_aligment* const sb = m.pool.data() + sw.first, * const se = sb + sw.count;
    const gaml_aligment* b = std::lower_bound(sb, se, *a, before);
    while (a < ae && b < se) {
      if (before(*a, *b)) a++;
      else if (before(*b, *a)) b++;
      else { drop[(size_t)(a - m.pool.data())] = 1; a++; }
    }
  }
}

static inline bool rec_before(const gaml_aligment& x, const gaml_aligment& y) { return x.position != y.position ? x.position < y.position : x.read_id < y.read_id; }
// ... 232 lines not shown

void OccImage::set_direct(int32_t w, const OccQuad& q) {
  const uint64_t e = occ8_pack(q, false);
  occ12[w] = Occ12{(uint32_t)e, (uint32_t)(e >> 32), q.rank};
  mark(w);
}

void OccImage::add_path(size_t n_windows, const std::vector<Occ>& occ, int32_t slot) {
  grow(n_windows);
  for (const Occ& o : occ) {
    const OccQuad q{o.shift, o.min_pos, slot, o.rank};
    const int32_t w = o.wid;
    if (cnt_[w] == 0) {
      cnt_[w] = 1;
      if (stamp_[w] != serial_) { stamp_[w] = serial_; touched_.push_back(w); }
      if (occ_fits_direct(q)) { set_direct(w, q); continue; }
      gen_[w].push_back(q);
    } else {
      auto it = gen_.find(w);
      if (it == gen_.end()) it = gen_.emplace(w, std::vector<OccQuad>(1, occ_from_direct(occ12[w]))).first;
      it->second.push_back(q);
      cnt_[w]++;
    }
    lists_dirty_ = true;
  }
}

void OccImage::remove_path(const std::vector<Occ>& occ, int32_t slot) {
  for (const Occ& o : occ) {
    const int32_t w = o.wid;
    if (w >= (int32_t)cnt_.size() || cnt_[w] == 0) continue;
    auto it = gen_.find(w);
    if (it == gen_.end()) {
      cnt_[w] = 0;
      occ12[w] = Occ12{~0u, ~0u, 0};
      mark(w);
      continue;
    }
    auto& lst = it->second;
    for (size_t k = 0; k < lst.size(); k++)
      if (lst[k].path == slot && lst[k].rank == o.rank && lst[k].shift == o.shift) { lst.erase(lst.begin() + k); break; }
    cnt_[w] = (int32_t)lst.size();
    lists_dirty_ = true;
    if (lst.empty()) { gen_.erase(it); occ12[w] = Occ12{~0u, ~0u, 0}; mark(w); }
    else if (lst.size() == 1 && occ_fits_direct(lst[0])) { const OccQuad q = lst[0]; gen_.erase(it); set_direct(w, q); }
  }
}

void OccImage::finalize(const std::vector<int32_t>& pos_of_slot) {
  if (!lists_dirty_) return;
  lists_dirty_ = false;
  lists_changed = true;
  multi_off.assign(1, 0);
  multi.clear();
  general_wids.clear();
  if (gen_.empty()) return;
  for (auto& e : gen_) general_wids.push_back(e.first);
  std::sort(general_wids.begin(), general_wids.end());
  for (int32_t w : general_wids) {
    auto& lst = gen_[w];
    std::sort(lst.begin(), lst.end(), [&](const OccQuad& x, const OccQuad& y) {
      const int32_t px = pos_of_slot[x.path], py = pos_of_slot[y.path];
      return px != py ? px < py : x.rank < y.rank;
    });
    const int32_t list = (int32_t)multi_off.size() - 1;
    multi.insert(multi.end(), lst.begin(), lst.end());
    multi_off.push_back((int32_t)multi.size());
    const uint64_t e = occ8_pack(OccQuad{0, 0, 0, 0}, true);
    const Occ12 ent{(uint32_t)e, (uint32_t)(e >> 32), -(list + 1)};
    if (occ12[w].lo != ent.lo || occ12[w].hi != ent.hi || occ12[w].rank != ent.rank) { occ12[w] = ent; mark(w); }
  }
}

void OccImage::dump(std::vector<Occ>& out) const {
  out.clear();
  for (size_t w = 0; w < cnt_.size(); w++) {
    if (cnt_[w] == 0) continue;
    auto it = gen_.find((int32_t)w);
    if (it == gen_.end()) { const OccQuad q = occ_from_direct(occ12[w]); out.push_back(Occ{(int32_t)w, q.shift, q.min_pos, q.path, q.rank}); }
    else for (const OccQuad& q : it->second) out.push_back(Occ{(int32_t)w, q.shift, q.min_pos, q.path, q.rank});
  }
}

void OccImage::build(size_t n_windows, const PlanView& view, int mate) {
  grow(n_windows);
  stale_.swap(touched_);
  touched_.clear();
  gen_.clear();
  if (++serial_ == 0) { std::fill(stamp_.begin(), stamp_.end(), 0); serial_ = 1; }
  for (size_t slot = 0; slot < view.paths.size(); slot++) {
    const PathMemo& pm = *view.paths[slot];
    const std::vector<OccPre>& pre = pm.pre[mate];
    const bool slot_fits = slot < 32767;
    const uint32_t slot_bits = (uint32_t)(slot & 0x7fff) << 16;
    for (size_t k = 0; k < pre.size(); k++) {
      const OccPre& e = pre[k];
      const bool direct = slot_fits && e.wid >= 0;
      const int32_t w = e.wid >= 0 ? e.wid : ~e.wid;
      if (stamp_[w] != serial_) {
        stamp_[w] = serial_; cnt_[w] = 1; touched_.push_back(w);
        if (direct) occ12[w] = Occ12{e.lo, e.hi | slot_bits, e.rank};
        else { const Occ& o = pm.occ[mate][k]; gen_[w].push_back(OccQuad{o.shift, o.min_pos, (int32_t)slot, o.rank}); }
        continue;
      }
      const Occ& o = pm.occ[mate][k];
      auto it = gen_.find(w);
      if (it == gen_.end()) it = gen_.emplace(w, std::vector<OccQuad>(1, occ_from_direct(occ12[w]))).first;
      it->second.push_back(OccQuad{o.shift, o.min_pos, (int32_t)slot, o.rank});
      cnt_[w]++;
    }
  }
  for (int32_t w : stale_) if (stamp_[w] != serial_ && cnt_[w]) { occ12[w] = Occ12{~0u, ~0u, 0}; cnt_[w] = 0; }
  changed_all = true;
  lists_dirty_ = true;
  std::vector<int32_t> ident(view.paths.size());
  for (size_t k = 0; k < ident.size(); k++) ident[k] = (int32_t)k;
  finalize(ident);
}

void build_occ_table(size_t n_windows, const std::vector<Occ>& occs, OccTable& out) {
  out.direct.assign(n_windows, OccQuad{0, 0, -1, 0});
  out.multi_off.assign(1, 0);
  out.multi.clear();
  std::vector<int32_t> cnt(n_windows, 0);
  for (const Occ& o : occs) cnt[o.wid]++;
  std::vector<int32_t> slot(n_windows, -1);
  for (const Occ& o : occs) if (cnt[o.wid] == 1 && (o.path >= 32767 || o.min_pos > 32767)) cnt[o.wid] = 1 << 30;
  for (const Occ& o : occs) {
    if (cnt[o.wid] == 1) { out.direct[o.wid] = OccQuad{o.shift, o.min_pos, o.path, o.rank}; continue; }
    if (cnt[o.wid] == (1 << 30)) cnt[o.wid] = 1;
    if (slot[o.wid] < 0) {
      slot[o.wid] = (int32_t)out.multi_off.size() - 1;
      out.multi_off.push_back(out.multi_off.back() + cnt[o.wid]);
      out.direct[o.wid] = OccQuad{0, 0, o.path, -(slot[o.wid] + 1)};
      cnt[o.wid] = -cnt[o.wid] - 2;
    }
  }
  out.multi.resize(out.multi_off.back());
  std::vector<int32_t> fill(out.multi_off.size(), 0);
  for (const Occ& o : occs) {
    if (slot[o.wid] < 0) continue;
    int32_t s = slot[o.wid];
    out.multi[out.multi_off[s] + fill[s]++] = OccQuad{o.shift, o.min_pos, o.path, o.rank};
  }
}

bool read_fastq(const std::string& file, std::string& bases, std::vector<int64_t>& offs, std::string* err,
                std::vector<std::string>* names) {
  std::ifstream f(file.c_str());
  if (!f.is_open()) { if (err) *err = "cannot open reads file " + file; return false; }
  std::unordered_map<std::string, int64_t> ids;
  std::vector<std::string> reads;
  std::string l, s;
  while (std::getline(f, l)) {
    std::string name = l.size() > 0 ? l.substr(1) : std::string();
    size_t cut = name.find_first_of(" \t");
    if (cut != std::string::npos) name.resize(cut);
    std::getline(f, s);
    auto it = ids.find(name);
    if (it == ids.end()) { ids.emplace(name, (int64_t)reads.size()); reads.push_back(s); if (names) names->push_back(name); }
    else reads[it->second] = s;
    std::getline(f, l);
    std::getline(f, l);
  }
  bases.clear();
  offs.assign(1, 0);
  for (auto& r : reads) { bases += r; offs.push_back((int64_t)bases.size()); }
  return true;
}

namespace {
inline int32_t atoi_range(const char* p, const char* e) {
  while (p < e && (*p == ' ' || (*p >= '\t' && *p <= '\r'))) p++;
  bool neg = false;
  if (p < e && (*p == '-' || *p == '+')) { neg = *p == '-'; p++; }
  int64_t v = 0;
  while (p < e && *p >= '0' && *p <= '9') { v = v * 10 + (*p - '0'); if (v > INT32_MAX) v = INT32_MAX; p++; }
  return (int32_t)(neg ? -v : v);
}
}

bool parse_sam_record(const char* b, const char* e, int32_t total_len, SamRecord& a) {
  thread_local std::vector<std::pair<const char*, const char*>> col;
  col.clear();
  for (const char* p = b;;) {
    const char* t = (const char*)memchr(p, '\t', (size_t)(e - p));
    if (!t) { col.emplace_back(p, e); break; }
    col.emplace_back(p, t);
    p = t + 1;
  }
  if (col.size() < 10) return false;
  auto num = [&](size_t i, size_t skip = 0) {
    return atoi_range(col[i].first + std::min<size_t>(skip, (size_t)(col[i].second - col[i].first)), col[i].second);
  };
  a.name.clear(); a.cigar.clear();
  {
    const char* cut = col[0].first;
// ... 142 lines not shown
```

gaml_amd/csrc/host_model.h:

```cpp
#pragma once
#include <climits>
#include <cstdint>
#include <memory>
#include <string>
#include <unordered_map>
#include <vector>

#include "../../include/gaml_hip.h"

namespace gaml {

constexpr int kTail = 300;
constexpr int kSeed = 15;

struct GraphStore {
  std::string bases;
  std::vector<int64_t> off;
  std::vector<int32_t> norm;
  int32_t n() const { return (int32_t)off.size() - 1; }
  int32_t len(int32_t node) const { return (int32_t)(off[node + 1] - off[node]); }
  const char* seq(int32_t node) const { return bases.data() + off[node]; }
  void finish();
  bool load_lastgraph(const std::string& file, std::string* err);
};
// ... 79 lines not shown
  std::vector<int32_t> pending;
  void cpu_align_records(const GraphStore& g, const Walk& w, std::vector<gaml_aligment>& recs) const;
  void finalize_window(int32_t wid, std::vector<gaml_aligment>& recs_sorted_local);
  void flush_pending_cpu(const GraphStore& g);
  std::string window_string(const GraphStore& g, const Walk& w, int32_t* offset) const;
};

struct Extension { int32_t errs, begin, end; };
bool extend_seed(int32_t win_pos, int32_t read_pos, const char* read, int32_t rlen, const char* win, int32_t wlen,
                 Extension* out);

void span_maxima(const char* s, int32_t n, int32_t read_len, std::vector<std::pair<uint64_t, int32_t>>& out);
uint64_t read_max_hash(const char* s, int32_t n);

void register_for_paths(const GraphStore& g, ShortMate& m, const std::vector<Walk>& paths);
void register_for_contig(const GraphStore& g, ShortMate& m, const int32_t* ctg, int32_t n);

struct Placement { int32_t wid, shift, path, contig, node; };
void placements_paired_contig(const GraphStore& g, const ShortMate& m, const int32_t* ctg, int32_t n, int32_t st,
                              int32_t path, int32_t contig_serial, std::vector<Placement>& out);
void occurrences_from_placements(ShortMate& m, const std::vector<Placement>& pl, std::vector<Occ>& out);
void occurrences_single_contig(const GraphStore& g, ShortMate& m, const int32_t* ctg, int32_t n, int32_t st,
                               int32_t* rank, std::vector<Occ>& out);

struct RecQuad { int32_t wid, pos, flags, link; };
struct ReadMajor {
  std::vector<RecQuad> first;
  std::vector<RecQuad> extra;
  uint64_t built_generation = ~0ull;
  int64_t total_records = 0;
};
void build_read_major(const ShortMate& m, const std::vector<int32_t>* slot_of_read, ReadMajor& out);
constexpr uint64_t kNoRec8 = ~0ull;
inline bool rec8_fits(int32_t wid, int32_t pos, int32_t edit) { return wid >= 0 && wid < (1 << 24) - 1 && pos >= 0 && pos < (1 << 28) && edit >= 0 && edit < 64; }
inline uint64_t rec8_pack(int32_t wid, int32_t pos, int32_t edit, int32_t orient) {
  return (uint64_t)(uint32_t)wid | ((uint64_t)(uint32_t)pos << 24) | ((uint64_t)(uint32_t)edit << 52) | ((uint64_t)(orient & 1) << 58);
}
#ifndef GAML_FOLD_CLASS2_BELOW
#define GAML_FOLD_CLASS2_BELOW 1024
#endif
constexpr int64_t kFoldClass2Below = GAML_FOLD_CLASS2_BELOW;
constexpr int kMemoCodes = 4;
constexpr int32_t kStaticZero = -2;
constexpr size_t kMemoMaxEntries = (size_t)1 << 24;
#ifdef GAML_HIP_DEV
struct PairTables {
  std::vector<int32_t> slot_of_read, read_of_slot;
  int64_t class_count[4] = {0, 0, 0, 0};
  int64_t n0a = 0;
  std::vector<int32_t> static_idx;
  std::vector<uint64_t> rec8[2];
  std::vector<uint8_t> len_code;
  std::vector<uint32_t> len_combo;
  std::vector<uint32_t> len12;
  ReadMajor rm[2];
  std::vector<RecQuad> inl[2];
  int64_t dropped_records[2] = {0, 0};
};
void build_pair_tables(const ShortMate& a, const ShortMate& b, PairTables& out, bool fold = true, int ins_n = 0);
#endif
void link_mate_windows(ShortMate& a, ShortMate& b);
#ifdef GAML_HIP_DEV
int64_t undominated_records(const ShortMate& m, int32_t wid, std::vector<uint8_t>& keep);
#endif


struct OccQuad { int32_t shift, min_pos, path, rank; };
struct OccTable {
  std::vector<OccQuad> direct;
  std::vector<int32_t> multi_off;
  std::vector<OccQuad> multi;
};
void build_occ_table(size_t n_windows, const std::vector<Occ>& occs, OccTable& out);

void split_contigs(const Walk& path, std::vector<std::pair<int32_t, int32_t>>& ctg_ranges, std::vector<int32_t>& gaps);

struct PlanView;
struct Occ12 { uint32_t lo, hi; int32_t rank; };
struct OccImage {
  std::vector<Occ12> occ12;
  std::vector<int32_t> multi_off;
  std::vector<OccQuad> multi;
  std::vector<int32_t> general_wids;
  void build(size_t n_windows, const PlanView& view, int mate);
  void add_path(size_t n_windows, const std::vector<Occ>& occ, int32_t slot);
  void remove_path(const std::vector<Occ>& occ, int32_t slot);
  void finalize(const std::vector<int32_t>& pos_of_slot);
  std::vector<int32_t> changed;
  bool changed_all = true, lists_changed = true;
  void dump(std::vector<Occ>& out) const;
  template <class F> void for_each_present(F f) const { for (int32_t w : touched_) if (cnt_[w] > 0) f(w); }
  void take_changed() { changed.clear(); changed_all = false; lists_changed = false; if (++mark_serial_ == 0) { std::fill(mark_.begin(), mark_.end(), 0); mark_serial_ = 1; } }
 private:
  void grow(size_t n_windows);
  void mark(int32_t w) { if (mark_[w] != mark_serial_) { mark_[w] = mark_serial_; changed.push_back(w); } }
  void set_direct(int32_t w, const OccQuad& q);
  std::vector<int32_t> touched_, stale_, cnt_, list_of_;
  std::vector<uint32_t> stamp_, mark_;
  uint32_t serial_ = 0, mark_serial_ = 1;
  struct Pending { int32_t wid; OccQuad q; };
  std::vector<Pending> pending_;
  std::unordered_map<int32_t, std::vector<OccQuad>> gen_;
  bool lists_dirty_ = false;
};

struct OccPre { int32_t wid; uint32_t lo, hi; int32_t rank; };

struct PathMemo {
  Walk path;
  bool registered[2] = {false, false};
  bool first_pending[2] = {false, false};
  bool valid[2] = {false, false};
  bool occ_valid[2] = {false, false};
  std::vector<Placement> pl[2];
  std::vector<Occ> occ[2];
  std::vector<OccPre> pre[2];
  int64_t assembled[2] = {0, 0};
  std::vector<int32_t> starts;
  int32_t length = 0;
  int32_t first_idx = -1, first_end = -1;
  int32_t final_last_end = -2;
  int32_t use_count = 0;
  uint32_t touched_serial = 0;
  uint64_t last_used = 0;
  uint32_t serial = 0;
};

struct PlanView {
  std::vector<const PathMemo*> paths;
};

class PairedPlanner {
 public:
  bool begin(const GraphStore& g, ShortMate mate[2], const int32_t* flat, const int64_t* offs, int32_t n_paths,
             bool allow_incremental, std::string* err);
  void finish(ShortMate mate[2]);
  void apply(ShortMate mate[2], OccImage image[2]);
  void mark_used(ShortMate mate[2], const OccImage image[2]);
  void note_rebuild(bool retired_some) { rebuild_clock_ = clock_; if (retired_some) retire_serial_++; }
  void invalidate_thresholds();
  void forget_previous() { have_prev_ = false; }
  const PlanView& view();
  void flat_occurrences(int mate, std::vector<Occ>& out);
  size_t memo_count() const { return memos_.size(); }
  int32_t total_len() const { return total_len_; }
  int64_t assembled(int mate) const { return assembled_[mate]; }
  int32_t n_paths() const { return (int32_t)cur_ids_.size(); }
  bool last_was_incremental() const { return incremental_; }
  const std::vector<int32_t>& slots() const { return cur_slots_; }
  uint64_t hits = 0, misses = 0, incremental_calls = 0, full_calls = 0;
 private:
  int32_t lookup_or_create(const GraphStore& g, const int32_t* p, int32_t len, std::string* err);
  void drain(ShortMate mate[2]);
  void build_placements(const GraphStore& g, ShortMate& m, int mt, PathMemo& pm, int32_t id);
  void registration_chain(const GraphStore& g, ShortMate mate[2], int32_t from, int32_t to);
  std::vector<std::unique_ptr<PathMemo>> memos_;
  std::unordered_map<Walk, int32_t, WalkHasher> by_path_;
  std::unordered_map<Walk, std::vector<std::pair<int32_t, uint32_t>>, WalkHasher> missed_[2];
  PlanView view_;
  bool view_valid_ = false;
  std::vector<int32_t> cur_ids_;
  std::vector<int32_t> cur_slots_;
  std::vector<int32_t> free_slots_, pos_of_slot_;
  int32_t next_slot_ = 0;
  std::vector<int32_t> prev_flat_;
  std::vector<int64_t> prev_offs_;
  bool have_prev_ = false;
  bool incremental_ = false;
  struct Removed { int32_t slot; int64_t assembled[2]; std::vector<Occ> occ[2]; };
  std::vector<Removed> removed_;
  std::vector<int32_t> work_;
  std::vector<int32_t> stale_;
  std::vector<char> redo_;
  struct Edit { int32_t p0, p1, c0, c1; };
  std::vector<Edit> edits_;
  std::vector<char> is_new_;
  int32_t total_len_ = 0;
  int64_t assembled_[2] = {0, 0};
  uint64_t clock_ = 0, rebuild_clock_ = 0;
  uint32_t retire_serial_ = 0;
  static constexpr size_t kMaxMemos = 2048;
};
int32_t walk_length(const GraphStore& g, const Walk& w);

bool read_fastq(const std::string& file, std::string& bases, std::vector<int64_t>& offs, std::string* err,
                std::vector<std::string>* names = nullptr);

struct SamRecord {
  std::string name;
  int32_t flags = 0, len = 0, posstart = 0, posend = 0, sstart = 0, send = 0, slen = 0, tstart = 0, tend = 0, edit_dist = 0;
  std::vector<std::pair<int32_t, char>> cigar;
};
bool parse_sam_record(const char* begin, const char* end, int32_t total_len, SamRecord& out);

struct DpBand {
  int32_t row0 = 0, max_width = 0;
  std::vector<int32_t> lo, hi;
};
void pacbio_dp_band(const std::vector<std::pair<int32_t, char>>& cigar, DpBand& out);

struct DpShape {
  int32_t n_ops = 0, row_f = 0, col_f = 0, bl = 0, el = 0, max_width = 0;
};
void pacbio_dp_ops(const std::vector<std::pair<int32_t, char>>& cigar, std::vector<uint32_t>& ops, DpShape& out);

}
```

gaml_amd/csrc/paired_launch.hip.h:

```cpp
#pragma once

namespace {

int paired_host_tabs(gaml_hip_ctx* c, PairedSet& s) {
  if (!s.ins_tab.empty() || !s.floor_tab.empty()) return 0;
  const double c0 = s.cfg.min_prob_start, k0 = s.cfg.min_prob_per_base;
  auto ins = [&](int d) {
    double z = ((double)d - s.cfg.insert_mean) / s.cfg.insert_std;
    return std::exp(-z * z / 2.0) / (std::sqrt(2 * M_PI) * s.cfg.insert_std);
  };
  const int kInsCap = 1 << 22;
  s.ins_tab.clear();
  for (int d = 0; d < kInsCap; d++) {
    double v = ins(d);
    if (v == 0.0 && (double)d > s.cfg.insert_mean) break;
    s.ins_tab.push_back(v);
  }
  if ((int)s.ins_tab.size() >= kInsCap)
    return fail(c, GAML_HIP_EINVAL, "insert_std too large: the insert-size table would exceed 4M entries");
  int smax = s.mate[0].max_len + s.mate[1].max_len;
  s.floor_tab.resize(smax + 1);
  s.logfloor_tab.resize(smax + 1);
  for (int v = 0; v <= smax; v++) {
    s.floor_tab[v] = std::exp(c0 + k0 * v);
    s.logfloor_tab[v] = std::log(s.floor_tab[v]);
    if (!(s.floor_tab[v] > 0.0)) s.floor_positive = false;
  }
  s.covthr_tab.resize(s.mate[1].max_len + 1);
  for (int v = 0; v <= s.mate[1].max_len; v++) s.covthr_tab[v] = std::exp(c0 + k0 * (v + v));
  return 0;
}

int prepare_paired_tables(gaml_hip_ctx* c, PairedSet& s) {
  if (s.tabs_uploaded) return 0;
  if (int e = paired_host_tabs(c, s)) return e;
  size_t total = s.ins_tab.size() + s.floor_tab.size() + s.logfloor_tab.size() + s.covthr_tab.size();
  HIP_TRY(c, s.tabs.reserve(std::max<size_t>(1, total) * sizeof(double)));
  double* d = s.tabs.as<double>();
  size_t at = 0;
  auto up = [&](const std::vector<double>& v) -> hipError_t {
    hipError_t e = v.empty() ? hipSuccess : hipMemcpy(d + at, v.data(), v.size() * sizeof(double), hipMemcpyHostToDevice);
    at += v.size();
    return e;
  };
  HIP_TRY(c, up(s.ins_tab));
  HIP_TRY(c, up(s.floor_tab));
  HIP_TRY(c, up(s.logfloor_tab));
  HIP_TRY(c, up(s.covthr_tab));
  const int64_t n = s.mate[0].n_local();
  HIP_TRY(c, s.probs.reserve(std::max<size_t>(1, n) * sizeof(double)));
  HIP_TRY(c, s.red.init());
  HIP_TRY(c, s.bad.reserve(sizeof(unsigned long long)));
  s.tabs_uploaded = true;
  return 0;
}

int prepare_paired_structure(gaml_hip_ctx* c, PairedSet& s, const int32_t* flat, const int64_t* offs, int32_t n_paths) {
  const bool incremental = !(s.cfg.penalty_constant > 0) && KNOB(c, 12) == 0;
  std::string err;
  if (!s.planner.begin(c->g, s.mate, flat, offs, n_paths, incremental, &err)) return fail(c, GAML_HIP_EINVAL, err);
  return 0;
}

void prepare_paired_tables_host(gaml_hip_ctx* c, PairedSet& s, PairedPrep& p) {
  (void)c;
  static const bool trace = getenv("GAML_HIP_TRACE_HOST") != nullptr;
  const double q0 = now_us();
  s.planner.finish(s.mate);
  const double q1 = now_us();
  const bool cov = s.cfg.penalty_constant > 0;
  p.path_base.assign(1, 0);
  p.start_off.assign(1, 0);
  p.starts.clear();
  if (cov) {
    const PlanView& v = s.planner.view();
    p.path_base.reserve(v.paths.size() + 1);
    p.start_off.reserve(v.paths.size() + 1);
    for (const PathMemo* pm : v.paths) {
      p.starts.insert(p.starts.end(), pm->starts.begin(), pm->starts.end());
      p.start_off.push_back((int32_t)p.starts.size());
      int32_t bits = ((pm->length + 64 + 31) / 32) * 32;
      p.path_base.push_back(p.path_base.back() + bits);
    }
  }
  p.total_bits = p.path_base.back();
  p.n_paths = s.planner.n_paths();
  const double q2 = now_us();
  s.planner.apply(s.mate, s.image);
  p.assembled_records = s.planner.assembled(0) + s.planner.assembled(1);
  p.general = !s.image[0].general_wids.empty() || !s.image[1].general_wids.empty();
  if (trace) fprintf(stderr, "pass2: finish %.1f us, starts %.1f us, images %.1f us\n", q1 - q0, q2 - q1, now_us() - q2);
}

}
#include "paired_tables.hip.h"
namespace {

double tfloor_for(double floor, double two_T) {
  if (!(floor > 0.0)) return 0.0;
  double x = floor * two_T;
  for (int k = 0; k < 64 && x > 0.0 && (std::nextafter(x, 0.0) / two_T) >= floor; k++) x = std::nextafter(x, 0.0);
  for (int k = 0; k < 64 && (x / two_T) < floor; k++) x = std::nextafter(x, std::numeric_limits<double>::infinity());
  return x;
}

struct PairedLayout { size_t tfloor_off; OccLayout l0, l1; size_t pb_off, so_off, st_off, total; };

PairedLayout paired_layout(const PairedSet& s, const PairedPrep& p, const size_t* pad_to = nullptr) {
  PairedLayout L;
  L.tfloor_off = 0;
  const size_t hdr = align16(256 * sizeof(double));
  L.l0 = layout_image(s.image[0], hdr, pad_to ? pad_to[0] : 0);
  L.l1 = layout_image(s.image[1], L.l0.end, pad_to ? pad_to[1] : 0);
  L.pb_off = L.l1.end; L.so_off = L.st_off = 0; L.total = L.l1.end;
  if (s.cfg.penalty_constant > 0) {
    L.so_off = align16(L.pb_off + p.path_base.size() * sizeof(int32_t));
    L.st_off = align16(L.so_off + p.start_off.size() * sizeof(int32_t));
    L.total = align16(L.st_off + p.starts.size() * sizeof(int32_t));
  }
  return L;
}

void paired_pack_thresholds(const PairedSet& s, const PairedLayout& L, double two_T, char* dst) {
  double tf[256];
  const size_t nc = std::min<size_t>(256, s.pt.len_combo.size());
  for (size_t ci = 0; ci < nc; ci++) {
    const int L0 = (int)(s.pt.len_combo[ci] & 0xffff), L1 = (int)(s.pt.len_combo[ci] >> 16);
    tf[ci] = tfloor_for(s.floor_tab[L0 + L1], two_T);
  }
  if (nc) memcpy(dst + L.tfloor_off, tf, nc * sizeof(double));
}

void paired_pack(const PairedSet& s, const PairedPrep& p, const PairedLayout& L, char* dst) {
  pack_image(s.image[0], L.l0, dst);
  pack_image(s.image[1], L.l1, dst);
  if (s.cfg.penalty_constant > 0) {
    memcpy(dst + L.pb_off, p.path_base.data(), p.path_base.size() * sizeof(int32_t));
    memcpy(dst + L.so_off, p.start_off.data(), p.start_off.size() * sizeof(int32_t));
    memcpy(dst + L.st_off, p.starts.data(), p.starts.size() * sizeof(int32_t));
  }
}

int arena_acquire(gaml_hip_ctx* c, Arena& A, size_t bytes, hipStream_t st, int* slot_out, char** write_ptr) {
  const int k = A.next;
  A.next = (A.next + 1) % kRing;
  if (A.armed[k]) { HIP_TRY(c, hipEventSynchronize(A.done[k])); A.armed[k] = false; }
  if (!A.done[k]) HIP_TRY(c, hipEventCreateWithFlags(&A.done[k], hipEventDisableTiming));
  const bool direct = c->direct_write && KNOB(c, 8) == 0;
  if (bytes > A.cap[k] || A.direct[k] != direct) {
    HIP_TRY(c, hipStreamSynchronize(st));
    if (A.dev[k]) { HIP_TRY(c, hipFree(A.dev[k])); A.dev[k] = nullptr; A.cap[k] = 0; }
    const size_t want = std::max<size_t>(bytes + bytes / 2, (size_t)1 << 20);
    if (direct) HIP_TRY(c, hipExtMallocWithFlags(&A.dev[k], want, hipDeviceMallocFinegrained));
    else HIP_TRY(c, hipMalloc(&A.dev[k], want));
    A.cap[k] = want; A.direct[k] = direct;
  }
  if (direct) *write_ptr = (char*)A.dev[k];
  else { HIP_TRY(c, A.host[k].reserve(bytes)); *write_ptr = (char*)A.host[k].p; }
  *slot_out = k;
  return 0;
}

int arena_commit(gaml_hip_ctx* c, Arena& A, int k, size_t bytes, hipStream_t st) {
  if (A.direct[k]) { _mm_sfence(); return 0; }
  if (bytes == 0) return 0;
  if (KNOB(c, 8) == 1 || (bytes & 15)) { HIP_TRY(c, hipMemcpyAsync(A.dev[k], A.host[k].p, bytes, hipMemcpyHostToDevice, st)); return 0; }
  const int n16 = (int)(bytes / 16);
  hipLaunchKernelGGL(stage_copy_kernel, dim3((unsigned)std::min(64, (n16 + kBlock - 1) / kBlock)), dim3(kBlock), 0, st,
                     (const int4*)A.host[k].dev, (int4*)A.dev[k], n16);
  HIP_TRY(c, hipGetLastError());
  return 0;
}

int arena_release(gaml_hip_ctx* c, Arena& A, int k, hipStream_t st) {
// ... 124 lines not shown
  const size_t nd = (size_t)s.nd_est;
  a.spill_slot = s.sp_slot.as<int>();
  a.dstate = s.dstate.as<int>();
  a.dirty_slots = s.dl_slot.as<int>();
  a.dirty_spill = s.dl_spill.as<int>();
  const int64_t ovf_total = n - n_main + s.ns_est + (s.spill_may_grow ? 4 : 0);
  const int64_t one_round = (n0a + 4 * kBlock - 1) / (4 * kBlock);
  const int cap0 = KNOB(c, 0) > 0 ? KNOB(c, 0)
                                   : (int)std::min<int64_t>(kMaxBlocks, one_round > 768 && one_round <= 1280 ? one_round : std::max<int64_t>(768, n0 / 2900));
  gp.blocks0a = n0a > 0 ? (int)std::max<int64_t>(1, std::min<int64_t>((n0a + 2 * kBlock - 1) / (2 * kBlock), cap0)) : 0;
  const int cap0b = KNOB(c, 20) > 0 ? KNOB(c, 20) : std::max(1, n0a > 0 ? cap0 / 3 : cap0);
  const int64_t blocks0b = n0b > 0 ? std::max<int64_t>(1, std::min<int64_t>(n0a > 0 ? (n0b + kBlock - 1) / kBlock : (n0b + 2 * kBlock - 1) / (2 * kBlock), cap0b)) : 0;
  gp.blocks0 = (int)std::max<int64_t>(1, gp.blocks0a + blocks0b);
  const int cap1 = KNOB(c, 10) > 0 ? KNOB(c, 10) : cap0 / 3;
  gp.blocks1 = (int)std::max<int64_t>(1, std::min<int64_t>((n01 - n0 + kBlock - 1) / kBlock, cap1));
  gp.blocks2 = (int)std::max<int64_t>(1, std::min<int64_t>((n_main - n01 + kBlock - 1) / kBlock, kMaxBlocks / 4));
  gp.blocks_d = nd ? (int)std::min<int64_t>(((int64_t)nd + kBlock - 1) / kBlock, 1024) : 0;
  gp.main_blocks = gp.blocks0 + gp.blocks1 + gp.blocks2 + gp.blocks_d;
  gp.ovf_blocks = ovf_total > 0 ? (int)std::min<int64_t>((ovf_total + 3) / 4, kOvfMaxBlocks) : 0;
  gp.total_blocks = gp.main_blocks + gp.ovf_blocks;
  a.blocks0a = gp.blocks0a;
  a.blocks0 = gp.blocks0;
  a.blocks01 = gp.blocks0 + gp.blocks1;
  a.blocks012 = gp.blocks0 + gp.blocks1 + gp.blocks2;
  a.main_blocks = gp.main_blocks;
  a.total_blocks = gp.total_blocks;
}

void paired_set_view(const PairedSet& s, const PairedLayout& L, const char* arena, int32_t total_len, SetDev& sd) {
  const OccLayout* l[2] = {&L.l0, &L.l1};
  for (int mt = 0; mt < 2; mt++) {
    sd.occ12[mt] = (const Occ12*)(arena + l[mt]->direct);
    sd.multi_off[mt] = (const int*)(arena + l[mt]->multi_off);
    sd.multi[mt] = (const int4*)(arena + l[mt]->multi);
  }
  sd.tfloor_c = (const double*)(arena + L.tfloor_off);
  const int tl = total_len == 0 ? 1 : total_len;
  sd.two_T = (double)(2 * tl);
  sd.tfloor0 = paired_tfloor0(s, sd.two_T);
  sd.log_two_T = std::log(sd.two_T);
  sd.part_sum = nullptr; sd.part_zero = nullptr;
}

void paired_apply_set(PairedArgs& a, const SetDev& sd) {
  for (int mt = 0; mt < 2; mt++) { a.m[mt].occ12 = sd.occ12[mt]; a.m[mt].occ = nullptr; a.occ12[mt] = sd.occ12[mt]; a.m[mt].multi_off = sd.multi_off[mt]; a.m[mt].multi = sd.multi[mt]; }
  a.tfloor_c = sd.tfloor_c; a.tfloor0 = sd.tfloor0; a.two_T = sd.two_T; a.log_two_T = sd.log_two_T;
  a.part_sum = sd.part_sum; a.part_zero = sd.part_zero;
}

CovArgs paired_cov_args(const PairedSet& s, const PairedPrep& p, const PairedLayout& L, const char* arena) {
  CovArgs ca;
  ca.bits = s.cov_bits.as<uint32_t>();
  ca.path_base = (const int*)(arena + L.pb_off);
  ca.start_off = (const int*)(arena + L.so_off);
  ca.starts = (const int*)(arena + L.st_off);
  ca.n_paths = p.n_paths;
  ca.total_words = p.total_bits / 32;
  ca.cov_move = s.cfg.step;
  ca.far = s.cfg.insert_mean + 5 * s.cfg.insert_std;
  ca.bad = s.bad.as<unsigned long long>();
  return ca;
}

int paired_host_partials(gaml_hip_ctx* c, PairedSet& s, int first_set, int n_sets, int n_partials, double** d_sum, int** d_zero) {
  const size_t per = (size_t)(4 * kMaxBlocks + kOvfMaxBlocks);
  HIP_TRY(c, s.h_part_sum.reserve(per * sizeof(double) * kMaxSets));
  HIP_TRY(c, s.h_part_zero.reserve(per * sizeof(int) * kMaxSets));
  *d_sum = (double*)s.h_part_sum.dev;
  *d_zero = (int*)s.h_part_zero.dev;
  double* hs = (double*)s.h_part_sum.p;
  int* hz = (int*)s.h_part_zero.p;
  for (int k = first_set; k < first_set + n_sets; k++) {
    for (int b2 = 0; b2 < n_partials; b2++) { hs[(size_t)k * per + b2] = std::numeric_limits<double>::quiet_NaN(); hz[(size_t)k * per + b2] = INT_MIN; }
    s.last_blocks[k] = n_partials;
  }
  s.host_part_stride = per;
  return 0;
}

int launch_paired(gaml_hip_ctx* c, PairedSet& s, PairedPrep& p, int32_t total_len, hipStream_t st, double* out4) {
  const double tpp = now_us();
  if (int e = prepare_paired_tables(c, s)) return e;
  const double tp0 = now_us();
  prepare_paired_tables_host(c, s, p);
  const double t_after_host = now_us();
  c->prof[1] = t_after_host - tp0;
  gpu_probe(st, c->warm_buf.p, "before table sync");
  if (int e = paired_sync_tables(c, s, st)) return e;
  const double tp1 = now_us();
  c->prof[4] = tp1 - t_after_host;
  if (tp1 - t_after_host > 1000.0 && getenv("GAML_HIP_TRACE_HOST")) fprintf(stderr, "table sync took %.0f us (evaluation %lld of the set, rebuild active %d slice %d)\n", tp1 - t_after_host, (long long)s.eval_count, (int)s.rebuild.active, s.rebuild.next_slice);

  const bool cov = s.cfg.penalty_constant > 0;
  const int tl = total_len == 0 ? 1 : total_len;
  const bool resident = c->host_results && c->direct_write && KNOB(c, 8) == 0 && KNOB(c, 13) == 0 && !cov;
  PairedLayout L;
  memset(&L, 0, sizeof(L));
  int slot = -1;
  const char* arena = nullptr;
  SetDev sd;
  if (resident) {
    c->prof[6] = (double)((s.image[0].changed_all || s.image[1].changed_all || !s.persist.valid) ? (s.image[0].occ12.size() + s.image[1].occ12.size()) * sizeof(Occ12)
                                                                                            : (s.image[0].changed.size() + s.image[1].changed.size()) * sizeof(Occ12));
    if (int e = paired_persist_update(c, s, (double)(2 * tl), st)) return e;
    paired_persist_view(s, total_len, sd);
  } else {
    L = paired_layout(s, p);
    char* wp = nullptr;
    if (int e = arena_acquire(c, s.arena, L.total, st, &slot, &wp)) return e;
    paired_pack(s, p, L, wp);
    paired_pack_thresholds(s, L, (double)(2 * tl), wp);
    if (int e = arena_commit(c, s.arena, slot, L.total, st)) return e;
    arena = (const char*)s.arena.dev[slot];
    paired_set_view(s, L, arena, total_len, sd);
    c->prof[6] = (double)L.total;
  }
  const double tp2 = now_us();
  c->prof[3] = tp2 - tp1;

  PairedArgs a;
  GridPlan gp;
  paired_base_args(c, s, a, gp);
  const int64_t n = s.mate[0].n_local();
  if (cov) {
    size_t words = (size_t)p.total_bits / 32;
    if (words * 4 > s.cov_bits.cap) { HIP_TRY(c, hipStreamSynchronize(st)); HIP_TRY(c, s.cov_bits.reserve(std::max<size_t>(4, words * 4))); }
    HIP_TRY(c, hipMemsetAsync(s.cov_bits.p, 0, std::max<size_t>(4, words * 4), st));
    HIP_TRY(c, hipMemsetAsync(s.bad.p, 0, sizeof(unsigned long long), st));
    a.cov_bits = s.cov_bits.as<uint32_t>();
    a.path_base = (const int*)(arena + L.pb_off);
  }
  const bool gen_set = a.n_main > 0 && p.general;
  const int n_partials = gp.total_blocks;
  sd.part_sum = s.red.part_sum.as<double>();
  sd.part_zero = s.red.part_zero.as<int>();
  if (c->host_results && n > 0) { if (int e = paired_host_partials(c, s, 0, 1, n_partials, &sd.part_sum, &sd.part_zero)) return e; }
  s.last_blocks[0] = n > 0 ? n_partials : 0;
  s.last_host_partials = c->host_results;
  s.last_sets = 1;
  paired_apply_set(a, sd);
  a.out = out4;
  a.timeline = nullptr;
  const bool timeline = KNOB(c, 3) == 8;
  if (timeline) {
    HIP_TRY(c, s.h_timeline.reserve((size_t)(4 * kMaxBlocks + kOvfMaxBlocks + 256) * (kBlock / 64) * 8 * sizeof(unsigned long long)));
    memset(s.h_timeline.p, 0, s.h_timeline.cap);
    a.timeline = (unsigned long long*)s.h_timeline.dev;
    s.timeline_waves = a.total_blocks * (kBlock / 64);
  }

  std::pair<hipEvent_t, hipEvent_t>* ev = nullptr;
  if (n > 0) {
    if (c->event_timing && (c->event_tick++ % c->event_every) == 0) { if (int e = take_events(c, &ev)) return e; }
    int fin_mode = c->host_results ? 2 : (KNOB(c, 2) ? KNOB(c, 2) - 1 : 1);
    double* status_out = nullptr;
    if (fin_mode != 2 && c->status_dst && !c->status_done) { status_out = c->status_dst; c->status_done = true; }
    if (fin_mode == 0) { a.status_out = status_out; a.status_a = c->status_a; a.status_b = c->status_b; }
    s.last_total_blocks = n_partials;
    const dim3 grid(a.total_blocks), block(kBlock);
    hipEvent_t e0 = ev ? ev->first : nullptr, e1 = ev ? ev->second : nullptr;
#define GAML_LAUNCH_SCORE(...) hipExtLaunchKernelGGL((paired_score_kernel<__VA_ARGS__>), grid, block, KNOB(c, 1), st, e0, e1, 0, a)
#ifdef GAML_HIP_DEV
    if (timeline) GAML_LAUNCH_SCORE(false, false, true);
    else
#endif
    if (gen_set) { if (fin_mode) GAML_LAUNCH_SCORE(false, true); else GAML_LAUNCH_SCORE(true, true); }
    else if (fin_mode) GAML_LAUNCH_SCORE(false, false);
    else GAML_LAUNCH_SCORE(true, false);
#undef GAML_LAUNCH_SCORE
    HIP_TRY(c, hipGetLastError());
    if (fin_mode == 1) {
      hipLaunchKernelGGL(finish_partials_kernel, dim3(1), dim3(kBlock), 0, st, a.part_sum, a.part_zero, n_partials, out4, cov ? -1.0 : 0.0, (double)n, status_out, c->status_a, c->status_b);
      HIP_TRY(c, hipGetLastError());
    }
  } else {
    s.last_total_blocks = 0;
    if (!c->host_results) HIP_TRY(c, hipMemsetAsync(out4, 0, 4 * sizeof(double), st));
  }
  if (cov && c->defer_cov) {
    int idx = 0;
    for (size_t i = 0; i < c->paireds.size(); i++) if (c->paireds[i].get() == &s) idx = (int)i;
    c->pending_cov.push_back(gaml_hip_ctx::PendingCov{idx, paired_cov_args(s, p, L, arena), out4});
  } else if (cov && n > 0 && p.total_bits > 0) {
    const CovArgs ca = paired_cov_args(s, p, L, arena);
// ... 71 lines not shown
```

include/gaml_hip_debug.h:

```cpp
#ifndef GAML_HIP_DEBUG_H_
#define GAML_HIP_DEBUG_H_

#include "gaml_hip.h"

#ifdef __cplusplus
extern "C" {
#endif

int gaml_hip_debug_sam_logprob(gaml_hip_ctx* ctx, const char* target, int32_t target_len, const char* read, int32_t read_len,
                               const char* sam_line, int64_t sam_len, double mismatch_prob, double* logprob_out,
                               int32_t* band_lo, int32_t* band_hi, int32_t band_cap);
int gaml_hip_debug_sam_shape(const char* sam_line, int64_t len, int32_t total_len, int32_t* out6, uint32_t* ops, int32_t cap);
int32_t gaml_hip_debug_sam_band(const char* sam_line, int64_t len, int32_t total_len, int32_t* fields10, int32_t* row0,
                                int32_t* lo, int32_t* hi, int32_t cap);

int gaml_hip_debug_prepare(gaml_hip_ctx* ctx, const int32_t* paths, const int64_t* path_offs, int32_t n_paths);
int64_t gaml_hip_debug_occurrences(gaml_hip_ctx* ctx, int readset, int mate, int32_t* out5, int64_t cap);
int64_t gaml_hip_debug_table_occurrences(gaml_hip_ctx* ctx, int readset, int mate, int32_t* out5, int64_t cap, int64_t* info3);
int32_t gaml_hip_debug_window_walk(gaml_hip_ctx* ctx, int readset, int mate, int32_t window_id, int32_t* out, int32_t cap);
int gaml_hip_debug_timeline(gaml_hip_ctx* ctx, int rs, unsigned long long* out, int64_t cap_waves);

int gaml_hip_debug_set_knob(gaml_hip_ctx* ctx, int knob, int value);
int gaml_hip_debug_fold_check(gaml_hip_ctx* ctx, int readset, int64_t* out6);
int gaml_hip_debug_radix_sort(gaml_hip_ctx* ctx, uint64_t* keys, uint64_t* vals, int64_t n, int begin_bit, int end_bit, uint64_t* run_max);
int gaml_hip_debug_static_check(gaml_hip_ctx* ctx, int readset, int64_t* out8);
int gaml_hip_debug_tables_check(gaml_hip_ctx* ctx, int readset, int64_t* out8);
int32_t gaml_hip_debug_block_partials(gaml_hip_ctx* ctx, int readset, int32_t set, double* sums, int32_t* zeros, int32_t cap, int32_t* layout8);

#ifdef __cplusplus
}
#endif
#endif
```

Before: 54.15 billion reads/s.

## Build occurrence tables on device from a resident pool of per-path prepacked entries

```diff
diff --git a/gaml_amd/api.py b/gaml_amd/api.py
--- a/gaml_amd/api.py
+++ b/gaml_amd/api.py
@@ -194,6 +194,10 @@
         L.gaml_hip_debug_static_check.argtypes = [vp, C.c_int, _i64p]
     if hasattr(L, "gaml_hip_debug_set_knob"):
         L.gaml_hip_debug_set_knob.argtypes = [vp, C.c_int, C.c_int]
+    if hasattr(L, "gaml_hip_debug_occ_route"):
+        L.gaml_hip_debug_occ_route.argtypes = [vp, C.c_int, _i64p]
+    if hasattr(L, "gaml_hip_debug_occ_check"):
+        L.gaml_hip_debug_occ_check.argtypes = [vp, C.c_int, _i64p]
     if hasattr(L, "gaml_hip_shm_exchange_open"):
         L.gaml_hip_shm_exchange_open.argtypes = [vp, C.c_char_p, C.c_int32, C.c_int32, C.c_int32]
         L.gaml_hip_shm_allreduce_sum.argtypes = [vp, C.c_void_p, C.c_int32]
@@ -686,6 +690,20 @@
         return {"static_pairs": int(out[0]), "other_pairs": int(out[1]), "violations": int(out[2]), "no_record": int(out[3]),
                 "different_windows": int(out[4]), "orientation": int(out[5]), "distance": int(out[6]), "edits_or_code": int(out[7])}
 
+    def debug_occ_route(self, rs):
+        out = np.zeros(6, np.int64)
+        self._check(_lib.gaml_hip_debug_occ_route(self._h, rs, out))
+        return {"device": int(out[0]), "host": int(out[1]), "fallbacks": int(out[2]), "compactions": int(out[3]),
+                "pool_entries": int(out[4]), "shared_combinations": int(out[5])}
+
+    def debug_occ_check(self, rs):
+        out = np.zeros(4, np.int64)
+        rc = _lib.gaml_hip_debug_occ_check(self._h, rs, out)
+        res = {"compared": int(out[0]), "present": int(out[1]), "mismatches": int(out[2]), "lists": int(out[3])}
+        if rc != 0 and res["compared"] == 0:
+            self._check(rc)
+        return res
+
     def debug_tables_check(self, rs):
         out = np.zeros(8, np.int64)
         rc = _lib.gaml_hip_debug_tables_check(self._h, rs, out)
diff --git a/gaml_amd/csrc/ctx.hip.h b/gaml_amd/csrc/ctx.hip.h
--- a/gaml_amd/csrc/ctx.hip.h
+++ b/gaml_amd/csrc/ctx.hip.h
@@ -268,6 +268,32 @@
     bool valid = false;
     void release() { if (dev) (void)hipFree(dev); dev = nullptr; bytes = 0; valid = false; }
   } persist;
+  struct OccDev {
+    DevBuf pool[2];
+    size_t pool_cap[2] = {0, 0}, pool_used[2] = {0, 0};
+    uint32_t pool_gen = 1;
+    PinBuf stage;
+    DevBuf tab[2][2], list[2][2];
+    DevBuf stamp[2];
+    size_t cap_w = 0, cap_list = 0;
+    int32_t list_n[2][2] = {{0, 0}, {0, 0}};
+    uint32_t serial = 0;
+    PinBuf dup;
+    bool taken = false;
+    bool check_dup = false;
+    bool image_stale = false;
+    std::vector<std::vector<uint64_t>> shared;
+    size_t shared_next = 0;
+    std::vector<uint64_t> key;
+    int64_t dev_calls = 0, host_calls = 0, fallbacks = 0, compactions = 0;
+    void release() {
+      for (int mt = 0; mt < 2; mt++) {
+        pool[mt].release(); stamp[mt].release();
+        for (int k = 0; k < 2; k++) { tab[mt][k].release(); list[mt][k].release(); }
+      }
+      stage.release(); dup.release();
+    }
+  } occdev;
   int64_t batches_patched = 0, batches_full = 0;
   size_t batch_slack = 0;
   hipEvent_t ev_tables = nullptr, ev_ovf = nullptr;
@@ -407,6 +433,7 @@
   bool used_default_stream = false;
   double* status_dst = nullptr; double status_a = 0, status_b = 0; bool status_done = false;
   bool host_results = false;
+  bool occ_route = false;
   bool defer_cov = false;
   struct PendingCov { int paired_idx; CovArgs args; double* out4; };
   std::vector<PendingCov> pending_cov;
diff --git a/gaml_amd/csrc/debug_api.hip.h b/gaml_amd/csrc/debug_api.hip.h
--- a/gaml_amd/csrc/debug_api.hip.h
+++ b/gaml_amd/csrc/debug_api.hip.h
@@ -16,7 +16,7 @@
       PairedSet& ps = *c->paireds[h.idx];
       if (int e = prepare_paired_structure(c, ps, flat, offs, n_paths)) return e;
       if (int e = align_pending_pair(c, ps)) return e;
-      prepare_paired_tables_host(c, ps, p);
+      if (int e = prepare_paired_tables_host(c, ps, p)) return e;
     }
   }
   if (c->peers == 1) {
@@ -46,6 +46,7 @@
   PairedSet& ps = *c->paireds[c->handles[rs].idx];
   if (info3) { info3[0] = ps.planner.last_was_incremental(); info3[1] = (int64_t)ps.planner.incremental_calls; info3[2] = (int64_t)ps.planner.full_calls; }
   std::vector<Occ> v;
+  paired_images_refresh(ps);
   ps.image[mate].dump(v);
   const std::vector<int32_t>& slots = ps.planner.slots();
   std::unordered_map<int32_t, int32_t> pos;
@@ -300,3 +301,42 @@
   T.release();
   return bad ? fail(c, GAML_HIP_ESTATE, "record tables: the device build differs from the host restatement") : GAML_HIP_OK;
 }
+
+int gaml_hip_debug_occ_route(gaml_hip_ctx* c, int rs, int64_t* out6) {
+  MULTI_SHARD0(c);
+  if (!c || !out6 || rs < 0 || rs >= (int)c->handles.size() || c->handles[rs].kind != 1) return fail(c, GAML_HIP_EINVAL, "bad arguments");
+  const PairedSet::OccDev& D = c->paireds[c->handles[rs].idx]->occdev;
+  out6[0] = D.dev_calls; out6[1] = D.host_calls; out6[2] = D.fallbacks; out6[3] = D.compactions;
+  out6[4] = (int64_t)(D.pool_used[0] + D.pool_used[1]); out6[5] = (int64_t)D.shared.size();
+  return GAML_HIP_OK;
+}
+
+int gaml_hip_debug_occ_check(gaml_hip_ctx* c, int rs, int64_t* out4) {
+  MULTI_SHARD0(c);
+  if (!c || !out4 || rs < 0 || rs >= (int)c->handles.size() || c->handles[rs].kind != 1) return fail(c, GAML_HIP_EINVAL, "bad arguments");
+  PairedSet& ps = *c->paireds[c->handles[rs].idx];
+  const PairedSet::OccDev& D = ps.occdev;
+  out4[0] = out4[1] = out4[2] = out4[3] = 0;
+  if (!D.image_stale) return GAML_HIP_OK;
+  HIP_TRY(c, hipSetDevice(c->device));
+  HIP_TRY(c, hipStreamSynchronize(c->stream));
+  const PlanView& v = ps.planner.view();
+  for (int mt = 0; mt < 2; mt++) {
+    OccImage im;
+    im.build(ps.mate[mt].wins.size(), v, mt);
+    const size_t n = im.occ12.size();
+    std::vector<Occ12> dev(n);
+    if (n) HIP_TRY(c, hipMemcpy(dev.data(), occdev_table(ps, mt), n * sizeof(Occ12), hipMemcpyDeviceToHost));
+    for (size_t w = 0; w < n; w++) {
+      const Occ12& h = im.occ12[w];
+      const Occ12& d = dev[w];
+      const bool absent = h.lo == ~0u && h.hi == ~0u;
+      out4[0]++;
+      if (!absent) out4[1]++;
+      if (absent ? (d.lo != ~0u || d.hi != ~0u) : (d.lo != h.lo || d.hi != h.hi || d.rank != h.rank)) out4[2]++;
+    }
+    if (!im.general_wids.empty()) out4[3]++;
+  }
+  if (out4[2] || out4[3]) return fail(c, GAML_HIP_ESTATE, "device occurrence tables differ from the host image");
+  return GAML_HIP_OK;
+}
diff --git a/gaml_amd/csrc/gaml_hip.hip b/gaml_amd/csrc/gaml_hip.hip
--- a/gaml_amd/csrc/gaml_hip.hip
+++ b/gaml_amd/csrc/gaml_hip.hip
@@ -204,6 +204,7 @@
 
 }
 
+#include "occ_device.hip.h"
 #include "paired_launch.hip.h"
 
 namespace {
@@ -465,7 +466,7 @@
                                     s->dl_rec[m].release(); s->sp_rng[m].release(); s->sp_rec[m].release(); }
       s->dl_slot.release(); s->dl_spill.release(); s->sp_slot.release(); s->dstate.release(); s->dl_bins.release(); s->dl_bin_count.release(); s->dl_blk_tot.release(); s->dl_wlist.release(); s->h_dstate.release(); s->lcode.release(); s->len_combo_dev.release(); s->combo_tabs.release(); s->memo.release();
       drop_stage(s->stage_pool); s->h_part_sum.release(); s->h_part_zero.release(); s->h_timeline.release();
-      s->probs.release(); s->tabs.release(); s->arena.release(); s->persist.release(); s->cov_bits.release(); s->bad.release(); if (s->ev_tables) (void)hipEventDestroy(s->ev_tables); if (s->ev_ovf) (void)hipEventDestroy(s->ev_ovf);
+      s->probs.release(); s->tabs.release(); s->arena.release(); s->persist.release(); s->occdev.release(); s->cov_bits.release(); s->bad.release(); if (s->ev_tables) (void)hipEventDestroy(s->ev_tables); if (s->ev_ovf) (void)hipEventDestroy(s->ev_ovf);
       s->red.release();
     }
     for (auto& s : c->pacbios) { s->d_lens.release(); s->rec_off.release(); s->rec_walk.release(); s->rec_logp.release(); s->walk_count.release(); s->logprobs.release(); s->red.release(); drop_stage(s->stage);
@@ -1002,7 +1003,26 @@
   void* dres = nullptr;
   HIP_TRY(c, hipHostGetDevicePointer(&dres, c->packed_host.p, 0));
   c->host_results = true;
+  c->occ_route = true;
   int e = evaluate(c, paths, offs, n_paths, dres, c->stream, total_len_out);
+  c->occ_route = false;
+  c->host_results = false;
+  if (e) return e;
+  if (int e2 = fetch_partials(c, partials_out)) return e2;
+  bool redo = false;
+  for (auto& ps : c->paireds) {
+    PairedSet::OccDev& D = ps->occdev;
+    if (!D.check_dup) continue;
+    D.check_dup = false;
+    if (*(volatile int*)D.dup.p == 0) continue;
+    occdev_note_shared(D);
+    D.fallbacks++;
+    redo = true;
+  }
+  if (!redo) return GAML_HIP_OK;
+  c->host_results = true;
+  c->pending_open = true;
+  e = eval_finish(c, dres, c->stream);
   c->host_results = false;
   if (e) return e;
   return fetch_partials(c, partials_out);
@@ -1031,14 +1051,16 @@
   if (spin) {
     const double deadline = t0 + 2e6;
     for (auto& ps : c->paireds) {
+      const volatile int* dup = ps->occdev.check_dup ? (const volatile int*)ps->occdev.dup.p : nullptr;
       for (int k = 0; k < ps->last_sets && spin; k++) {
         const volatile double* hs = (const volatile double*)ps->h_part_sum.p + (size_t)k * ps->host_part_stride;
         const volatile int* hz = (const volatile int*)ps->h_part_zero.p + (size_t)k * ps->host_part_stride;
         int done = 0;
+        unsigned polls = 0;
         while (done < ps->last_blocks[k]) {
           if (hs[done] == hs[done] && hz[done] != INT_MIN) { done++; continue; }
           __builtin_ia32_pause();
-          if ((done & 63) == 0 && now_us() > deadline) { spin = false; break; }
+          if ((++polls & 63) == 0 && ((dup && *dup) || now_us() > deadline)) { spin = false; break; }
         }
       }
       if (!spin) break;
@@ -1132,6 +1154,7 @@
   if (c->device < 0) return fail(c, GAML_HIP_ENODEVICE, "scoring needs a HIP device: this context is host-only");
   if (n_sets == 0) return GAML_HIP_OK;
   HIP_TRY(c, hipSetDevice(c->device));
+  for (auto& ps : c->paireds) paired_images_refresh(*ps);
   const size_t ns = std::max<size_t>(1, c->handles.size());
   for (int32_t i = 0; i < n_sets; i++) if (set_offs[i + 1] < set_offs[i]) return fail(c, GAML_HIP_EINVAL, "set offsets must not decrease");
   int32_t done_sets = 0;
diff --git a/gaml_amd/csrc/host_model.cc b/gaml_amd/csrc/host_model.cc
--- a/gaml_amd/csrc/host_model.cc
+++ b/gaml_amd/csrc/host_model.cc
@@ -859,6 +859,13 @@
   }
 }
 
+static bool occ_pre_plain(const std::vector<OccPre>& pre) {
+  std::vector<int32_t> w(pre.size());
+  for (size_t k = 0; k < pre.size(); k++) { if (pre[k].wid < 0) return false; w[k] = pre[k].wid; }
+  std::sort(w.begin(), w.end());
+  return std::adjacent_find(w.begin(), w.end()) == w.end();
+}
+
 void PairedPlanner::invalidate_thresholds() {
   for (auto& pm : memos_) pm->occ_valid[0] = pm->occ_valid[1] = false;
   have_prev_ = false;
@@ -873,6 +880,8 @@
       pm.assembled[mt] = 0;
       for (const Occ& o : pm.occ[mt]) pm.assembled[mt] += mate[mt].wins[o.wid].count;
       occ_prepack(pm.occ[mt], pm.pre[mt]);
+      pm.pre_plain[mt] = occ_pre_plain(pm.pre[mt]);
+      pm.dev_off[mt] = -1;
       pm.occ_valid[mt] = true;
     }
   };
@@ -894,7 +903,7 @@
   return view_;
 }
 
-void PairedPlanner::apply(ShortMate mate[2], OccImage image[2]) {
+void PairedPlanner::apply(ShortMate mate[2], OccImage image[2], bool build_image, bool image_stale) {
   if (!incremental_) {
     const PlanView& v = view();
     for (int32_t id : cur_ids_) {
@@ -903,7 +912,21 @@
       for (int mt = 0; mt < 2; mt++) for (const Occ& o : pm.occ[mt]) mate[mt].touch(o.wid);
       pm.touched_serial = retire_serial_;
     }
-    for (int mt = 0; mt < 2; mt++) image[mt].build(mate[mt].wins.size(), v, mt);
+    if (build_image) for (int mt = 0; mt < 2; mt++) image[mt].build(mate[mt].wins.size(), v, mt);
+    return;
+  }
+  if (image_stale) {
+    for (int mt = 0; mt < 2; mt++) {
+      for (const Removed& r : removed_) assembled_[mt] -= r.assembled[mt];
+      for (int32_t k : work_) assembled_[mt] += memos_[cur_ids_[k]]->assembled[mt];
+    }
+    for (int32_t id : cur_ids_) {
+      PathMemo& pm = *memos_[id];
+      if (pm.touched_serial == retire_serial_) continue;
+      for (int mt = 0; mt < 2; mt++) for (const Occ& o : pm.occ[mt]) mate[mt].touch(o.wid);
+      pm.touched_serial = retire_serial_;
+    }
+    rebuild_images(mate, image);
     return;
   }
   for (int32_t k : work_) {
@@ -924,6 +947,13 @@
     }
     im.finalize(pos_of_slot_);
   }
+}
+
+void PairedPlanner::rebuild_images(ShortMate mate[2], OccImage image[2]) {
+  if ((int32_t)pos_of_slot_.size() < next_slot_) pos_of_slot_.resize((size_t)next_slot_ + 64, 0);
+  for (int32_t k = 0; k < (int32_t)cur_slots_.size(); k++) pos_of_slot_[cur_slots_[k]] = k;
+  const PlanView& v = view();
+  for (int mt = 0; mt < 2; mt++) image[mt].build(mate[mt].wins.size(), v, mt, &cur_slots_, &pos_of_slot_);
 }
 
 void PairedPlanner::mark_used(ShortMate mate[2], const OccImage image[2]) {
@@ -1322,14 +1352,16 @@
   }
 }
 
-void OccImage::build(size_t n_windows, const PlanView& view, int mate) {
+void OccImage::build(size_t n_windows, const PlanView& view, int mate, const std::vector<int32_t>* slots,
+                     const std::vector<int32_t>* pos_of_slot) {
   grow(n_windows);
   stale_.swap(touched_);
   touched_.clear();
   gen_.clear();
   if (++serial_ == 0) { std::fill(stamp_.begin(), stamp_.end(), 0); serial_ = 1; }
-  for (size_t slot = 0; slot < view.paths.size(); slot++) {
-    const PathMemo& pm = *view.paths[slot];
+  for (size_t pos = 0; pos < view.paths.size(); pos++) {
+    const PathMemo& pm = *view.paths[pos];
+    const size_t slot = slots ? (size_t)(*slots)[pos] : pos;
     const std::vector<OccPre>& pre = pm.pre[mate];
     const bool slot_fits = slot < 32767;
     const uint32_t slot_bits = (uint32_t)(slot & 0x7fff) << 16;
@@ -1353,6 +1385,7 @@
   for (int32_t w : stale_) if (stamp_[w] != serial_ && cnt_[w]) { occ12[w] = Occ12{~0u, ~0u, 0}; cnt_[w] = 0; }
   changed_all = true;
   lists_dirty_ = true;
+  if (pos_of_slot) { finalize(*pos_of_slot); return; }
   std::vector<int32_t> ident(view.paths.size());
   for (size_t k = 0; k < ident.size(); k++) ident[k] = (int32_t)k;
   finalize(ident);
diff --git a/gaml_amd/csrc/host_model.h b/gaml_amd/csrc/host_model.h
--- a/gaml_amd/csrc/host_model.h
+++ b/gaml_amd/csrc/host_model.h
@@ -185,7 +185,8 @@
   std::vector<int32_t> multi_off;
   std::vector<OccQuad> multi;
   std::vector<int32_t> general_wids;
-  void build(size_t n_windows, const PlanView& view, int mate);
+  void build(size_t n_windows, const PlanView& view, int mate, const std::vector<int32_t>* slots = nullptr,
+             const std::vector<int32_t>* pos_of_slot = nullptr);
   void add_path(size_t n_windows, const std::vector<Occ>& occ, int32_t slot);
   void remove_path(const std::vector<Occ>& occ, int32_t slot);
   void finalize(const std::vector<int32_t>& pos_of_slot);
@@ -218,6 +219,9 @@
   std::vector<Placement> pl[2];
   std::vector<Occ> occ[2];
   std::vector<OccPre> pre[2];
+  bool pre_plain[2] = {false, false};
+  int64_t dev_off[2] = {-1, -1};
+  uint32_t dev_gen[2] = {0, 0};
   int64_t assembled[2] = {0, 0};
   std::vector<int32_t> starts;
   int32_t length = 0;
@@ -238,7 +242,10 @@
   bool begin(const GraphStore& g, ShortMate mate[2], const int32_t* flat, const int64_t* offs, int32_t n_paths,
              bool allow_incremental, std::string* err);
   void finish(ShortMate mate[2]);
-  void apply(ShortMate mate[2], OccImage image[2]);
+  void apply(ShortMate mate[2], OccImage image[2], bool build_image = true, bool image_stale = false);
+  void rebuild_images(ShortMate mate[2], OccImage image[2]);
+  const std::vector<int32_t>& ids() const { return cur_ids_; }
+  PathMemo& memo(int32_t id) { return *memos_[id]; }
   void mark_used(ShortMate mate[2], const OccImage image[2]);
   void note_rebuild(bool retired_some) { rebuild_clock_ = clock_; if (retired_some) retire_serial_++; }
   void invalidate_thresholds();
diff --git a/gaml_amd/csrc/occ_device.hip.h b/gaml_amd/csrc/occ_device.hip.h
--- /dev/null
+++ b/gaml_amd/csrc/occ_device.hip.h
@@ -0,0 +1,196 @@
+#pragma once
+
+namespace {
+
+constexpr int kOccMaxDesc = 32;
+
+struct OccDesc { long long off; int slot, start; };
+struct OccScatterArgs {
+  const OccPre* pool[2];
+  Occ12* dst[2];
+  int* dst_list[2];
+  Occ12* clr[2];
+  const int* clr_list[2];
+  unsigned* stamp[2];
+  int* dup;
+  int n_desc, total[2], n_clr[2];
+  unsigned serial;
+  OccDesc desc[2][kOccMaxDesc];
+};
+
+__global__ void __launch_bounds__(kBlock) occ_scatter_kernel(const OccScatterArgs a) {
+  const int t0 = a.total[0], t01 = t0 + a.total[1], c0 = t01 + a.n_clr[0], n = c0 + a.n_clr[1];
+  for (int i = blockIdx.x * blockDim.x + threadIdx.x; i < n; i += gridDim.x * blockDim.x) {
+    if (i < t01) {
+      const int mt = i < t0 ? 0 : 1;
+      const int j = mt ? i - t0 : i;
+      int d = 0;
+      while (d + 1 < a.n_desc && a.desc[mt][d + 1].start <= j) d++;
+      const OccDesc& D = a.desc[mt][d];
+      const OccPre e = a.pool[mt][D.off + (j - D.start)];
+      Occ12* o = a.dst[mt] + e.wid;
+      o->lo = e.lo; o->hi = e.hi | ((unsigned)D.slot << 16); o->rank = e.rank;
+      a.dst_list[mt][j] = e.wid;
+      if (atomicExch(a.stamp[mt] + e.wid, a.serial) == a.serial) *(volatile int*)a.dup = 1;
+    } else {
+      const int mt = i < c0 ? 0 : 1;
+      const int j = mt ? i - c0 : i - t01;
+      Occ12* o = a.clr[mt] + a.clr_list[mt][j];
+      o->lo = ~0u; o->hi = ~0u; o->rank = -1;
+    }
+  }
+}
+
+bool paired_resident_route(const gaml_hip_ctx* c, const PairedSet& s) {
+  return c->host_results && c->direct_write && KNOB(c, 8) == 0 && KNOB(c, 13) == 0 && !(s.cfg.penalty_constant > 0);
+}
+
+bool occdev_route_ok(const gaml_hip_ctx* c, PairedSet& s) {
+  PairedSet::OccDev& D = s.occdev;
+  if (!c->occ_route || KNOB(c, 17) != 0 || !paired_resident_route(c, s) || !s.persist.valid) return false;
+  if (s.planner.last_was_incremental()) return false;
+  const std::vector<int32_t>& ids = s.planner.ids();
+  if (ids.empty() || ids.size() > (size_t)kOccMaxDesc) return false;
+  D.key.clear();
+  for (int32_t id : ids) {
+    const PathMemo& pm = s.planner.memo(id);
+    if (!pm.pre_plain[0] || !pm.pre_plain[1]) return false;
+    D.key.push_back((uint64_t)(uint32_t)id << 32 | pm.serial);
+  }
+  for (const auto& k : D.shared) if (k == D.key) return false;
+  return true;
+}
+
+void occdev_note_shared(PairedSet::OccDev& D) {
+  constexpr size_t kShared = 16;
+  if (D.shared.size() < kShared) D.shared.push_back(D.key);
+  else { D.shared[D.shared_next] = D.key; D.shared_next = (D.shared_next + 1) % kShared; }
+}
+
+int occdev_reserve(gaml_hip_ctx* c, PairedSet& s, size_t n_windows, size_t n_occ, hipStream_t st) {
+  PairedSet::OccDev& D = s.occdev;
+  if (D.cap_w > 0 && n_windows <= D.cap_w && n_occ <= D.cap_list) return 0;
+  HIP_TRY(c, hipStreamSynchronize(st));
+  D.cap_w = std::max(std::max<size_t>(4 * n_windows, (size_t)1 << 18), D.cap_w);
+  D.cap_list = std::max(std::max<size_t>(2 * n_occ, (size_t)1 << 16), D.cap_list);
+  for (int mt = 0; mt < 2; mt++) {
+    for (int k = 0; k < 2; k++) {
+      HIP_TRY(c, D.tab[mt][k].reserve(D.cap_w * sizeof(Occ12)));
+      HIP_TRY(c, hipMemsetAsync(D.tab[mt][k].p, 0xff, D.cap_w * sizeof(Occ12), st));
+      HIP_TRY(c, D.list[mt][k].reserve(D.cap_list * sizeof(int32_t)));
+      D.list_n[mt][k] = 0;
+    }
+    HIP_TRY(c, D.stamp[mt].reserve(D.cap_w * sizeof(uint32_t)));
+    HIP_TRY(c, hipMemsetAsync(D.stamp[mt].p, 0, D.cap_w * sizeof(uint32_t), st));
+  }
+  D.serial = 0;
+  return 0;
+}
+
+int occdev_upload(gaml_hip_ctx* c, PairedSet& s, hipStream_t st, size_t* bytes) {
+  PairedSet::OccDev& D = s.occdev;
+  const std::vector<int32_t>& ids = s.planner.ids();
+  auto missing = [&](const PathMemo& pm, int mt) { return pm.dev_off[mt] < 0 || pm.dev_gen[mt] != D.pool_gen; };
+  size_t need[2] = {0, 0}, whole[2] = {0, 0};
+  for (int32_t id : ids)
+    for (int mt = 0; mt < 2; mt++) { const PathMemo& pm = s.planner.memo(id); whole[mt] += pm.pre[mt].size(); if (missing(pm, mt)) need[mt] += pm.pre[mt].size(); }
+  if (D.pool_used[0] + need[0] > D.pool_cap[0] || D.pool_used[1] + need[1] > D.pool_cap[1]) {
+    HIP_TRY(c, hipStreamSynchronize(st));
+    for (int mt = 0; mt < 2; mt++) {
+      if (2 * whole[mt] > D.pool_cap[mt]) {
+        D.pool_cap[mt] = std::max<size_t>(8 * whole[mt], 2 * D.pool_cap[mt]);
+        HIP_TRY(c, D.pool[mt].reserve(D.pool_cap[mt] * sizeof(OccPre)));
+      }
+      D.pool_used[mt] = 0;
+      need[mt] = whole[mt];
+    }
+    D.pool_gen++;
+    D.compactions++;
+  }
+  *bytes = (need[0] + need[1]) * sizeof(OccPre);
+  if (need[0] + need[1] == 0) return 0;
+  HIP_TRY(c, D.stage.reserve(*bytes));
+  OccPre* sp = (OccPre*)D.stage.p;
+  for (int mt = 0; mt < 2; mt++) {
+    const size_t at = D.pool_used[mt];
+    size_t k = 0;
+    for (int32_t id : ids) {
+      PathMemo& pm = s.planner.memo(id);
+      if (!missing(pm, mt)) continue;
+      pm.dev_off[mt] = (int64_t)(at + k);
+      pm.dev_gen[mt] = D.pool_gen;
+      if (!pm.pre[mt].empty()) memcpy(sp + k, pm.pre[mt].data(), pm.pre[mt].size() * sizeof(OccPre));
+      k += pm.pre[mt].size();
+    }
+    if (k) HIP_TRY(c, hipMemcpyAsync(D.pool[mt].as<OccPre>() + at, sp, k * sizeof(OccPre), hipMemcpyHostToDevice, st));
+    D.pool_used[mt] = at + k;
+    sp += k;
+  }
+  return 0;
+}
+
+int occdev_launch(gaml_hip_ctx* c, PairedSet& s, hipStream_t st, size_t* bytes) {
+  PairedSet::OccDev& D = s.occdev;
+  const std::vector<int32_t>& ids = s.planner.ids();
+  if (D.pool_cap[0] == 0 || D.pool_cap[1] == 0) {
+    for (int mt = 0; mt < 2; mt++) {
+      size_t all = 0;
+      for (int32_t id : ids) all += s.planner.memo(id).pre[mt].size();
+      D.pool_cap[mt] = std::max<size_t>(16 * all, (size_t)1 << 10);
+      HIP_TRY(c, D.pool[mt].reserve(D.pool_cap[mt] * sizeof(OccPre)));
+      D.pool_used[mt] = 0;
+    }
+    D.pool_gen++;
+  }
+  size_t n_occ[2] = {0, 0};
+  for (int32_t id : ids) for (int mt = 0; mt < 2; mt++) n_occ[mt] += s.planner.memo(id).pre[mt].size();
+  const size_t n_windows = std::max(s.mate[0].wins.size(), s.mate[1].wins.size());
+  if (int e = occdev_reserve(c, s, n_windows, std::max(n_occ[0], n_occ[1]), st)) return e;
+  if (int e = occdev_upload(c, s, st, bytes)) return e;
+  HIP_TRY(c, D.dup.reserve(sizeof(int)));
+  *(volatile int*)D.dup.p = 0;
+  if (++D.serial == 0) {
+    for (int mt = 0; mt < 2; mt++) HIP_TRY(c, hipMemsetAsync(D.stamp[mt].p, 0, D.cap_w * sizeof(uint32_t), st));
+    D.serial = 1;
+  }
+  const int cur = (int)(D.serial & 1), other = cur ^ 1;
+  OccScatterArgs a;
+  memset(&a, 0, sizeof(a));
+  a.n_desc = (int)ids.size();
+  for (int mt = 0; mt < 2; mt++) {
+    a.pool[mt] = D.pool[mt].as<OccPre>();
+    a.dst[mt] = D.tab[mt][cur].as<Occ12>();
+    a.dst_list[mt] = D.list[mt][cur].as<int>();
+    a.clr[mt] = D.tab[mt][other].as<Occ12>();
+    a.clr_list[mt] = D.list[mt][other].as<int>();
+    a.stamp[mt] = D.stamp[mt].as<unsigned>();
+    int start = 0;
+    for (size_t k = 0; k < ids.size(); k++) {
+      const PathMemo& pm = s.planner.memo(ids[k]);
+      a.desc[mt][k] = OccDesc{(long long)pm.dev_off[mt], (int)k, start};
+      start += (int)pm.pre[mt].size();
+    }
+    a.total[mt] = start;
+    a.n_clr[mt] = D.list_n[mt][other];
+    D.list_n[mt][cur] = start;
+    D.list_n[mt][other] = 0;
+  }
+  a.dup = (int*)D.dup.dev;
+  a.serial = D.serial;
+  const int items = a.total[0] + a.total[1] + a.n_clr[0] + a.n_clr[1];
+  if (items > 0) {
+    hipLaunchKernelGGL(occ_scatter_kernel, dim3((unsigned)std::min(512, (items + kBlock - 1) / kBlock)), dim3(kBlock), 0, st, a);
+    HIP_TRY(c, hipGetLastError());
+  }
+  return 0;
+}
+
+const Occ12* occdev_table(const PairedSet& s, int mt) { return s.occdev.tab[mt][s.occdev.serial & 1].as<Occ12>(); }
+
+void paired_images_refresh(PairedSet& s) {
+  if (!s.occdev.image_stale) return;
+  s.planner.rebuild_images(s.mate, s.image);
+  s.occdev.image_stale = false;
+}
+
+}
diff --git a/gaml_amd/csrc/paired_launch.hip.h b/gaml_amd/csrc/paired_launch.hip.h
--- a/gaml_amd/csrc/paired_launch.hip.h
+++ b/gaml_amd/csrc/paired_launch.hip.h
@@ -62,11 +62,15 @@
   return 0;
 }
 
-void prepare_paired_tables_host(gaml_hip_ctx* c, PairedSet& s, PairedPrep& p) {
-  (void)c;
+int prepare_paired_tables_host(gaml_hip_ctx* c, PairedSet& s, PairedPrep& p, hipStream_t st = nullptr, bool device_route = false) {
   static const bool trace = getenv("GAML_HIP_TRACE_HOST") != nullptr;
   const double q0 = now_us();
   s.planner.finish(s.mate);
+  PairedSet::OccDev& D = s.occdev;
+  D.taken = device_route && occdev_route_ok(c, s);
+  size_t up_bytes = 0;
+  if (D.taken) { if (int e = occdev_launch(c, s, st, &up_bytes)) return e; }
+  c->prof[6] = (double)up_bytes;
   const double q1 = now_us();
   const bool cov = s.cfg.penalty_constant > 0;
   p.path_base.assign(1, 0);
@@ -86,10 +90,13 @@
   p.total_bits = p.path_base.back();
   p.n_paths = s.planner.n_paths();
   const double q2 = now_us();
-  s.planner.apply(s.mate, s.image);
+  s.planner.apply(s.mate, s.image, !D.taken, D.image_stale);
+  D.image_stale = D.taken;
+  if (D.taken) D.dev_calls++; else D.host_calls++;
   p.assembled_records = s.planner.assembled(0) + s.planner.assembled(1);
-  p.general = !s.image[0].general_wids.empty() || !s.image[1].general_wids.empty();
+  p.general = !D.taken && (!s.image[0].general_wids.empty() || !s.image[1].general_wids.empty());
   if (trace) fprintf(stderr, "pass2: finish %.1f us, starts %.1f us, images %.1f us\n", q1 - q0, q2 - q1, now_us() - q2);
+  return 0;
 }
 
 }
@@ -380,7 +387,7 @@
   const double tpp = now_us();
   if (int e = prepare_paired_tables(c, s)) return e;
   const double tp0 = now_us();
-  prepare_paired_tables_host(c, s, p);
+  if (int e = prepare_paired_tables_host(c, s, p, st, true)) return e;
   const double t_after_host = now_us();
   c->prof[1] = t_after_host - tp0;
   gpu_probe(st, c->warm_buf.p, "before table sync");
@@ -391,13 +398,22 @@
 
   const bool cov = s.cfg.penalty_constant > 0;
   const int tl = total_len == 0 ? 1 : total_len;
-  const bool resident = c->host_results && c->direct_write && KNOB(c, 8) == 0 && KNOB(c, 13) == 0 && !cov;
+  const bool resident = paired_resident_route(c, s);
   PairedLayout L;
   memset(&L, 0, sizeof(L));
   int slot = -1;
   const char* arena = nullptr;
   SetDev sd;
-  if (resident) {
+  s.occdev.check_dup = s.occdev.taken;
+  if (s.occdev.taken) {
+    PairedLayout Lt;
+    Lt.tfloor_off = s.persist.off_tfloor;
+    paired_pack_thresholds(s, Lt, (double)(2 * tl), (char*)s.persist.dev);
+    _mm_sfence();
+    paired_persist_view(s, total_len, sd);
+    for (int mt = 0; mt < 2; mt++) sd.occ12[mt] = occdev_table(s, mt);
+    c->prof[6] += 256.0 * sizeof(double);
+  } else if (resident) {
     c->prof[6] = (double)((s.image[0].changed_all || s.image[1].changed_all || !s.persist.valid) ? (s.image[0].occ12.size() + s.image[1].occ12.size()) * sizeof(Occ12)
                                                                                             : (s.image[0].changed.size() + s.image[1].changed.size()) * sizeof(Occ12));
     if (int e = paired_persist_update(c, s, (double)(2 * tl), st)) return e;
diff --git a/include/gaml_hip_debug.h b/include/gaml_hip_debug.h
--- a/include/gaml_hip_debug.h
+++ b/include/gaml_hip_debug.h
@@ -27,6 +27,9 @@
 int gaml_hip_debug_tables_check(gaml_hip_ctx* ctx, int readset, int64_t* out8);
 int32_t gaml_hip_debug_block_partials(gaml_hip_ctx* ctx, int readset, int32_t set, double* sums, int32_t* zeros, int32_t cap, int32_t* layout8);
 
+int gaml_hip_debug_occ_route(gaml_hip_ctx* ctx, int readset, int64_t* out6);
+int gaml_hip_debug_occ_check(gaml_hip_ctx* ctx, int readset, int64_t* out4);
+
 #ifdef __cplusplus
 }
 #endif
```

New measurement: 66.48 billion reads/s, median of 6. +22.8%, better.
